# google-research/swirl-fem

Hardware: AMD Instinct MI355X
Metric: GDOF/s per CG iteration, 3D p=7 Laplacian (higher is better)
Workload: dtype f64

## Files before the change

include/sfem.h:

```cpp
#ifndef SFEM_H_
#define SFEM_H_

#include <stdint.h>

#ifdef __cplusplus
extern "C" {
#endif

#define SFEM_ABI_VERSION 10

enum { SFEM_F32 = 0, SFEM_F64 = 1 };
enum {
  SFEM_OK = 0,
  SFEM_EINVAL = -1,
  SFEM_EHIP = -2,
  SFEM_EUNSUPPORTED = -3
};
#define SFEM_SENTINEL (-1)
#define SFEM_MAX_P 16

#define SFEM_IDX_MASK 0x3FFFFFFF
#define SFEM_IDX_PAD 0x3FFFFFFF
#define SFEM_IDX_DIRICHLET 0x80000000u
#define SFEM_IDX_SHARED 0x40000000u
// ... 300 lines not shown

#define SFEM_CG_NSCALARS_NAMED 16
#define SFEM_CG_RR_SLOTS 64
#define SFEM_CG_NSCALARS (SFEM_CG_NSCALARS_NAMED + SFEM_CG_RR_SLOTS)
#define SFEM_CG_MEAN_SUMS (4 * SFEM_CG_RR_SLOTS)
#define SFEM_CG_STATUS_RUNNING 0.0
#define SFEM_CG_STATUS_CONVERGED 1.0
#define SFEM_CG_STATUS_MAXITER 2.0
#define SFEM_CG_STATUS_BAD_PAP 3.0
#define SFEM_CG_STATUS_BAD_GAMMA 4.0
int sfem_dot(const void* a, const void* b, int64_t count, double* result,
             int dtype, sfem_stream_t stream);
int sfem_dot_accumulate(const void* a, const void* b, int64_t count,
                        double* result, int dtype, sfem_stream_t stream);
int sfem_dot_indexed(const void* a, const void* b, const int64_t* idx,
                     const double* w, int64_t count, int ncomp,
                     int64_t node_stride, int64_t comp_stride, double scale,
                     double* result, int dtype, sfem_stream_t stream);
int sfem_subtract_weighted_mean(const void* w, const void* b, double total,
                                void* out, double* partials, int64_t count,
                                double* dot_result, int dtype,
                                sfem_stream_t stream);
int sfem_cg_scalars(double* scalars, int phase, double maxiter, double tol,
                    double atol, double* partials, sfem_stream_t stream);
int sfem_cg_update_xr(void* x, void* r, const void* p, const void* ap,
                      int64_t count, double* scalars, int fuse_rr, int dtype,
                      sfem_stream_t stream);
int sfem_cg_update_p(void* p, const void* z, int64_t count, double* scalars,
                     int dtype, sfem_stream_t stream);
int sfem_cg_update_r(void* r, const void* ap, int64_t count, double* scalars,
                     int fuse_rr, int dtype, sfem_stream_t stream);
int sfem_cg_update_xp(void* x, void* p, const void* z, int64_t count,
                      double* scalars, int dtype, sfem_stream_t stream);
#define SFEM_FOLD_GROUPS 256
int sfem_cg_scalars_n(double* scalars, int phase, double maxiter, double tol,
                      double atol, double* partials, int64_t num_partials,
                      sfem_stream_t stream);
int sfem_cg_update_r_layered_det(void* r, const void* ap_ext, int64_t count,
                                 const int64_t* layer_len,
                                 const int64_t* layer_off, int num_layers,
                                 const uint8_t* layer_masks,
                                 const int64_t* mask_off,
                                 double* scalars, double* rr_partials,
                                 int64_t rr_capacity, int64_t* num_rr,
                                 int dtype, sfem_stream_t stream);
#define SFEM_CG_LAZY_MAX 8
int sfem_cg_update_xp_lazy(void* x, void* pring, int64_t ring_stride,
                           const void* z, int64_t count, double* scalars,
                           double* lazy, int m, int dtype,
                           sfem_stream_t stream);
int sfem_cg_flush_x(void* x, const void* pring, int64_t ring_stride,
                    int64_t count, const double* scalars, double* lazy, int m,
                    int dtype, sfem_stream_t stream);
#define SFEM_MAX_LAYERS 15
#define SFEM_LAYER_CHUNK 512
int sfem_cg_update_r_layered(void* r, const void* ap_ext, int64_t count,
                             const int64_t* layer_len,
                             const int64_t* layer_off, int num_layers,
                             const uint8_t* layer_masks,
                             const int64_t* mask_off, double* scalars,
                             int fuse_rr, int dtype, sfem_stream_t stream);
int sfem_fold_layers(void* out_ext, int64_t count, const int64_t* layer_len,
                     const int64_t* layer_off, int num_layers, int dtype,
                     sfem_stream_t stream);
int sfem_fold_layers_at(void* out_ext, const int64_t* idx, int64_t num_idx,
                        int64_t count, const int64_t* layer_len,
                        const int64_t* layer_off, int num_layers, int dtype,
                        sfem_stream_t stream);
int sfem_cg_update_r_mean(void* r, const void* ap, const void* w,
                          int64_t count, double* scalars, double* sums,
                          int dtype, sfem_stream_t stream);
int sfem_cg_update_xp_mean(void* x, void* p, const void* r, int64_t count,
                           double* scalars, double* sums, double total,
                           int dtype, sfem_stream_t stream);
int sfem_fdm_solve(const void* r, void* z, const int64_t* pel, const void* S,
                   const int32_t* cases, const void* inv_eigenvalues,
                   int64_t num_elements, int ndim, int Pp, int dtype,
                   sfem_stream_t stream);
int sfem_fdm_solve_sums(const void* r, void* z, const int64_t* pel,
                        const void* S, const int32_t* cases,
                        const void* inv_eigenvalues, const void* weights,
                        void* elem_sum, void* weighted_sum,
                        int64_t num_elements, int ndim, int Pp, int dtype,
                        sfem_stream_t stream);
int sfem_add_element_constants(void* z, const void* yc, const void* shift,
                               int64_t num_elements, int n,
                               int64_t elems_per_member, int dtype,
                               sfem_stream_t stream);
int sfem_ell_chebyshev(const int32_t* cols, const void* vals, const void* dinv,
                       const void* b, void* x, void* work, int64_t n,
                       int width, int steps, double lmin, double lmax,
                       int dtype, sfem_stream_t stream);
#define SFEM_ENS_NSCALARS 16
#define SFEM_ENS_GROUPS 32
#define SFEM_ENS_MAX_MEMBERS 4096
int sfem_ens_dot(const void* a, const void* b, int64_t len, int members,
                 double* partials, int which, int dtype, sfem_stream_t stream);
int sfem_ens_init(double* scalars, const double* partials, int members,
                  double maxiter, double tol, double atol,
                  sfem_stream_t stream);
int sfem_ens_update_r(void* r, const void* ap, int64_t len, int members,
                      const double* scalars, const double* partials,
                      int dtype, sfem_stream_t stream);
int sfem_ens_close(double* scalars, const double* partials, int members,
                   double maxiter, sfem_stream_t stream);
int sfem_ens_update_xp(void* x, void* p, const void* z, int64_t len,
// ... 124 lines not shown
```

swirl_fem_amd/_lib.py:

```python

from __future__ import annotations

import ctypes
import os

from swirl_fem_amd import switches

_HERE = os.path.dirname(os.path.abspath(__file__))
LIB_PATH = switches.get('SFEM_LIB') or os.path.join(_HERE, 'libsfem_hip.so')
ABI_VERSION = 10

SFEM_F32, SFEM_F64 = 0, 1
SFEM_CG_NSCALARS_NAMED = 16
SFEM_CG_NSCALARS = 80
SFEM_BICGSTAB_NSCALARS = 32
BICGSTAB_STATUS = {0: 'running', 1: 'converged', 2: 'maxiter',
                   3: 'breakdown_rho', 4: 'breakdown_omega',
                   5: 'breakdown_alpha'}
CG_STATUS = {0: 'running', 1: 'converged', 2: 'maxiter', 3: 'breakdown_pAp',
             4: 'breakdown_gamma'}
SFEM_DOT_SLOTS = 1024
SFEM_CG_MEAN_SUMS = 256
SFEM_MAX_LAYERS = 15
SFEM_FOLD_GROUPS = 256
# ... 176 lines not shown
    'sfem_helmholtz_sens': [ctypes.POINTER(HelmholtzSensArgs), c_ptr],
    'sfem_facet_table_build': [c_ptr, c_ptr, c_ptr, c_ptr, c_ptr, c_i64, c_i64,
                               c_i32, c_ptr],
    'sfem_helmholtz_setup_affine': [c_ptr, c_ptr, c_i64, c_dbl, c_i32, c_ptr],
    'sfem_helmholtz_cluster_limits': [c_i32, c_i32, ctypes.POINTER(c_i32),
                                      ctypes.POINTER(c_i32)],
    'sfem_dot': [c_ptr, c_ptr, c_i64, c_ptr, c_i32, c_ptr],
    'sfem_dot_accumulate': [c_ptr, c_ptr, c_i64, c_ptr, c_i32, c_ptr],
    'sfem_dot_indexed': [c_ptr, c_ptr, c_ptr, c_ptr, c_i64, c_i32, c_i64,
                         c_i64, c_dbl, c_ptr, c_i32, c_ptr],
    'sfem_cg_scalars': [c_ptr, c_i32, c_dbl, c_dbl, c_dbl, c_ptr, c_ptr],
    'sfem_cg_update_xr': [c_ptr, c_ptr, c_ptr, c_ptr, c_i64, c_ptr, c_i32,
                          c_i32, c_ptr],
    'sfem_cg_update_p': [c_ptr, c_ptr, c_i64, c_ptr, c_i32, c_ptr],
    'sfem_cg_update_r': [c_ptr, c_ptr, c_i64, c_ptr, c_i32, c_i32, c_ptr],
    'sfem_cg_update_xp': [c_ptr, c_ptr, c_ptr, c_i64, c_ptr, c_i32, c_ptr],
    'sfem_cg_update_r_layered': [c_ptr, c_ptr, c_i64, c_ptr, c_ptr, c_i32,
                                 c_ptr, c_ptr, c_ptr, c_i32, c_i32, c_ptr],
    'sfem_kernarg_selftest': [c_ptr, c_ptr],
    'sfem_fdm_solve': [c_ptr, c_ptr, c_ptr, c_ptr, c_ptr, c_ptr, c_i64, c_i32,
                       c_i32, c_i32, c_ptr],
    'sfem_fdm_solve_sums': [c_ptr, c_ptr, c_ptr, c_ptr, c_ptr, c_ptr, c_ptr,
                            c_ptr, c_ptr, c_i64, c_i32, c_i32, c_i32, c_ptr],
    'sfem_add_element_constants': [c_ptr, c_ptr, c_ptr, c_i64, c_i32, c_i64,
                                   c_i32, c_ptr],
    'sfem_ell_chebyshev': [c_ptr, c_ptr, c_ptr, c_ptr, c_ptr, c_ptr, c_i64,
                           c_i32, c_i32, c_dbl, c_dbl, c_i32, c_ptr],
    'sfem_ens_dot': [c_ptr, c_ptr, c_i64, c_i32, c_ptr, c_i32, c_i32, c_ptr],
    'sfem_ens_init': [c_ptr, c_ptr, c_i32, c_dbl, c_dbl, c_dbl, c_ptr],
    'sfem_ens_update_r': [c_ptr, c_ptr, c_i64, c_i32, c_ptr, c_ptr, c_i32,
                          c_ptr],
    'sfem_ens_close': [c_ptr, c_ptr, c_i32, c_dbl, c_ptr],
    'sfem_ens_update_xp': [c_ptr, c_ptr, c_ptr, c_i64, c_i32, c_ptr, c_i32,
                           c_ptr],
    'sfem_ens_update_r_mean': [c_ptr, c_ptr, c_ptr, c_i64, c_i32, c_ptr, c_ptr,
                               c_ptr, c_i32, c_ptr],
    'sfem_ens_close_mean': [c_ptr, c_ptr, c_ptr, c_dbl, c_i32, c_dbl, c_ptr],
    'sfem_ens_update_xp_mean': [c_ptr, c_ptr, c_ptr, c_i64, c_i32, c_ptr,
                                c_i32, c_ptr],
    'sfem_ens_subtract_weighted_mean': [c_ptr, c_ptr, c_dbl, c_ptr, c_ptr,
                                        c_i64, c_i32, c_i32, c_ptr],
    'sfem_fold_layers': [c_ptr, c_i64, c_ptr, c_ptr, c_i32, c_i32, c_ptr],
    'sfem_fold_layers_at': [c_ptr, c_ptr, c_i64, c_i64, c_ptr, c_ptr, c_i32,
                            c_i32, c_ptr],
    'sfem_cg_scalars_n': [c_ptr, c_i32, c_dbl, c_dbl, c_dbl, c_ptr, c_i64,
                          c_ptr],
    'sfem_cg_update_r_layered_det': [c_ptr, c_ptr, c_i64, c_ptr, c_ptr, c_i32,
                                     c_ptr, c_ptr, c_ptr, c_ptr, c_i64, c_ptr,
                                     c_i32, c_ptr],
    'sfem_cg_update_xp_lazy': [c_ptr, c_ptr, c_i64, c_ptr, c_i64, c_ptr, c_ptr,
                               c_i32, c_i32, c_ptr],
    'sfem_cg_flush_x': [c_ptr, c_ptr, c_i64, c_i64, c_ptr, c_ptr, c_i32, c_i32,
                        c_ptr],
    'sfem_cg_update_r_mean': [c_ptr, c_ptr, c_ptr, c_i64, c_ptr, c_ptr, c_i32,
                              c_ptr],
    'sfem_cg_update_xp_mean': [c_ptr, c_ptr, c_ptr, c_i64, c_ptr, c_ptr, c_dbl,
                               c_i32, c_ptr],
    'sfem_axpby': [c_dbl, c_ptr, c_dbl, c_ptr, c_i64, c_i32, c_ptr],
    'sfem_helmholtz_diag': [ctypes.POINTER(DiagArgs), c_ptr],
    'sfem_cg_update_r_jacobi': [c_ptr, c_ptr, c_ptr, c_i64, c_i32, c_ptr,
                                c_ptr, c_i32, c_ptr, c_ptr, c_ptr, c_ptr,
                                c_i64, c_ptr, c_i32, c_ptr],
    'sfem_cg_update_xp_jacobi': [c_ptr, c_ptr, c_ptr, c_ptr, c_i64, c_i32,
                                 c_ptr, c_i32, c_ptr],
    'sfem_stokes_setup': [c_ptr, c_ptr, c_ptr, c_ptr, c_i64, c_i32, c_i32,
                          c_i32, c_ptr],
    'sfem_stokes_div': [c_ptr, c_ptr],
    'sfem_stokes_grad_t': [c_ptr, c_ptr],
    'sfem_stokes_e_first': [c_ptr, c_ptr],
    'sfem_stokes_e_second': [c_ptr, c_ptr],
    'sfem_stokes_convect_local': [c_ptr, c_ptr],
    'sfem_transport_rhs': [ctypes.POINTER(TransportArgs), c_ptr],
    'sfem_transport_rhs_vjp': [ctypes.POINTER(TransportVjpArgs), c_ptr],
    'sfem_point_locate': [ctypes.POINTER(PointLocateArgs), c_ptr],
    'sfem_point_eval': [ctypes.POINTER(PointArgs), c_ptr],
    'sfem_point_eval_t': [ctypes.POINTER(PointArgs), c_ptr],
    'sfem_pmg_prolong': [c_ptr, c_ptr, c_ptr, c_ptr, c_ptr, c_ptr, c_i64,
                         c_i32, c_i32, c_i32, c_i32, c_i32, c_ptr],
    'sfem_pmg_restrict': [c_ptr, c_ptr, c_ptr, c_ptr, c_ptr, c_ptr, c_i64,
                          c_i32, c_i32, c_i32, c_i32, c_ptr],
    'sfem_cheb_step': [c_ptr, c_ptr, c_ptr, c_ptr, c_ptr, c_ptr, c_dbl, c_dbl,
                       c_i64, c_i32, c_i32, c_ptr],
    'sfem_pmg_dot2': [c_ptr, c_ptr, c_ptr, c_i64, c_ptr, c_i32, c_i32, c_ptr],
    'sfem_pmg_cg_scalars': [c_ptr, c_i32, c_ptr, c_i64, c_dbl, c_dbl, c_dbl,
                            c_ptr],
    'sfem_boundary_geom': [c_ptr, c_ptr, c_i64, c_ptr, c_ptr, c_ptr, c_i32,
                           c_i32, c_i32, c_ptr, c_ptr, c_i32, c_ptr],
    'sfem_boundary_covector': [c_ptr, c_i32, c_ptr, c_i64, c_ptr, c_ptr,
                               c_i32, c_i32, c_i32, c_ptr, c_i32, c_ptr],
    'sfem_boundary_mass_apply': [c_ptr, c_ptr, c_i64, c_ptr, c_ptr, c_i32,
                                 c_i32, c_i32, c_dbl, c_ptr, c_i32, c_ptr],
    'sfem_boundary_mass_diag': [c_ptr, c_i64, c_ptr, c_ptr, c_i32, c_i32,
                                c_i32, c_dbl, c_ptr, c_i32, c_ptr],
    'sfem_boundary_add_rows': [c_ptr, c_ptr, c_ptr, c_ptr, c_i64, c_ptr, c_i32,
                               c_ptr],
    'sfem_ell_spmv': [c_ptr, c_ptr, c_ptr, c_ptr, c_i64, c_i32, c_i64, c_i64,
                      c_ptr, c_i64, c_i32, c_ptr],
    'sfem_bicgstab_scalars': [c_ptr, c_i32, c_dbl, c_dbl, c_dbl, c_ptr],
    'sfem_bicgstab_dot': [c_ptr, c_ptr, c_i64, c_ptr, c_i32, c_i32, c_i32,
                          c_ptr],
    'sfem_bicgstab_update_p': [c_ptr, c_ptr, c_ptr, c_ptr, c_ptr, c_i64, c_ptr,
                               c_i32, c_ptr],
    'sfem_bicgstab_update_s': [c_ptr, c_ptr, c_ptr, c_ptr, c_ptr, c_i64, c_ptr,
                               c_i32, c_ptr],
    'sfem_bicgstab_update_xr': [c_ptr, c_ptr, c_ptr, c_ptr, c_ptr, c_ptr,
                                c_ptr, c_i64, c_ptr, c_i32, c_ptr],
# ... 38 lines not shown
```

swirl_fem_amd/_ops.py:

```python

from __future__ import annotations

import ctypes
import os

import numpy as np
import torch

from swirl_fem_amd import switches
from swirl_fem_amd import _lib

_DT = {torch.float32: _lib.SFEM_F32, torch.float64: _lib.SFEM_F64}


def _dtype_code(t: torch.Tensor) -> int:
  try:
    return _DT[t.dtype]
  except KeyError:
    raise TypeError(f'unsupported dtype {t.dtype}; use float32 or float64')


def _dev(*tensors):
  dev = None
  for t in tensors:
# ... 499 lines not shown
    return 'sfem::helmholtz_mfma_p12_kernel<%d, %s>' % (geo_mode, b(mass))
  if part.get('cluster') is not None:
    return 'sfem::helmholtz_cluster_kernel<%s, %d, %s, %d, %s>' % (
        real, P, b(scalar), geo_mode, b(mass))
  if part.get('beta') is not None:
    return 'sfem::helmholtz_adv_kernel<%s, %d, %d, true, %d, false>' % (
        real, P, ndim, geo_mode)
  if part.get('coef_mode'):
    return ('sfem::helmholtz_kernel<%s, %d, %d, true, true, %d, false, %s, '
            '%d>' % (real, P, ndim, geo_mode, b(mass), part['coef_mode']))
  tpe = P * P if ndim == 3 else P
  can_sort = ndim == 3 and tpe <= 64
  sort = (can_sort and part.get('shared_order') is not None and
          not part.get('colored') and not (geo_mode == 3 and mass))
  b = lambda v: 'true' if v else 'false'
  return 'sfem::helmholtz_kernel<%s, %d, %d, true, %s, %d, %s, %s>' % (
      real, P, ndim, b(scalar), geo_mode, b(sort), b(mass))


def helmholtz_apply(u, out, enc, parts, host, ndim, P, lambda0, lambda1,
                    zero_range, dot_out=None, transpose=False):
  dev = _dev(enc)
  _check_vector_layout(u, out)
  host = {k: _host(v, u.dtype) for k, v in host.items()}
  if not parts and zero_range[1] > zero_range[0]:
    out[zero_range[0]:zero_range[1]].zero_()
  with torch.cuda.device(dev):
    for n, part in enumerate(parts):
      args = _helmholtz_args(u, out, part.get('enc', enc), part, host, ndim,
                             P, enc.shape[0], u.shape[0], lambda0, lambda1,
                             zero_range if n == 0 else (0, 0), dot_out,
                             transpose=transpose)
      _lib.check(_lib.load().sfem_helmholtz_apply(ctypes.byref(args),
                                                  _stream(dev)),
                 'sfem_helmholtz_apply')
  return out


def layered_dot_waves(parts, P, num_elements):
  waves = (P * P + 63) // 64
  out = []
  for part in parts:
    if part.get('layered_chains'):
      groups = part['chains'][0].numel() - 1
    elif 'elem_list' in part:
      groups = part['elem_list'].numel()
    else:
      groups = num_elements
    out.append(groups * waves)
  return out


def helmholtz_apply_layered(u, ext, enc, parts, host, ndim, P, lambda0,
                            lambda1, dot_out=None, per_wave=False):
  dev = _dev(enc)
  if u.dim() != 1 or not u.is_contiguous() or not ext.is_contiguous():
    raise ValueError('layered assembly takes contiguous scalar fields')
  if ext.dtype != u.dtype:
    raise ValueError('u and the extended output differ in dtype')
  host = {k: _host(v, u.dtype) for k, v in host.items()}
  waves = (layered_dot_waves(parts, P, enc.shape[0])
           if per_wave and dot_out is not None else None)
  if waves is not None and sum(waves) > dot_out.numel():
    raise ValueError(f'{sum(waves)} waves but {dot_out.numel()} dot slots')
  at = 0
  with torch.cuda.device(dev):
    for n, part in enumerate(parts):
      dots = dot_out if waves is None else dot_out[at:at + waves[n]]
      args = _helmholtz_args(u, ext, enc, part, host, ndim, P, enc.shape[0],
                             u.shape[0], lambda0, lambda1, (0, 0), dots,
                             layered_extent=ext.numel(),
                             dot_slots=0 if waves is None else waves[n])
      if waves is not None:
        at += waves[n]
      _lib.check(_lib.load().sfem_helmholtz_apply(ctypes.byref(args),
                                                  _stream(dev)),
                 'sfem_helmholtz_apply')
  return ext


def _layer_arrays(layers):
  n = len(layers)
  arr = ctypes.c_int64 * max(n, 1)
  return (arr(*[int(l[0]) for l in layers]) if n else arr(0),
          arr(*[int(l[1]) for l in layers]) if n else arr(0), n)


def _mask_args(masks, n):
  if masks is None:
    return None, None
  data, offs = masks
  arr = ctypes.c_int64 * max(n, 1)
  return _ptr(data), arr(*[int(o) for o in offs])


def cg_update_r_layered(r, ap_ext, layers, scalars, fuse_rr, masks=None):
  dev = _dev(r, ap_ext, scalars)
  ln, off, n = _layer_arrays(layers)
  mptr, moff = _mask_args(masks, n)
  with torch.cuda.device(dev):
    _lib.check(_lib.load().sfem_cg_update_r_layered(
        _ptr(r), _ptr(ap_ext), r.numel(), ln, off, n, mptr, moff,
        _ptr(scalars), int(fuse_rr), _dtype_code(r), _stream(dev)),
        'sfem_cg_update_r_layered')


def cg_update_r_layered_det(r, ap_ext, layers, scalars, rr_partials,
                            masks=None):
  dev = _dev(r, ap_ext, scalars, rr_partials)
  ln, off, n = _layer_arrays(layers)
  mptr, moff = _mask_args(masks, n)
  count = ctypes.c_int64(0)
  with torch.cuda.device(dev):
    _lib.check(_lib.load().sfem_cg_update_r_layered_det(
        _ptr(r), _ptr(ap_ext), r.numel(), ln, off, n, mptr, moff,
        _ptr(scalars),
        _ptr(rr_partials), rr_partials.numel(), ctypes.byref(count),
        _dtype_code(r), _stream(dev)), 'sfem_cg_update_r_layered_det')
  return count.value


def cg_scalars_n(scalars, phase, maxiter, tol, atol, partials, num_partials):
  dev = _dev(scalars, partials)
  with torch.cuda.device(dev):
    _lib.check(_lib.load().sfem_cg_scalars_n(
        _ptr(scalars), phase, float(maxiter), float(tol), float(atol),
        _ptr(partials), int(num_partials), _stream(dev)), 'sfem_cg_scalars_n')
# ... 688 lines not shown
  fn = (_lib.load().sfem_dot_accumulate if accumulate
        else _lib.load().sfem_dot)
  with torch.cuda.device(dev):
    _lib.check(fn(_ptr(a), _ptr(b), a.numel(),
                  ctypes.c_void_p(result.data_ptr() + 8 * slot),
                  _dtype_code(a), _stream(dev)), 'sfem_dot')


def dot_indexed(a, b, idx, w, result, slot, scale):
  ncomp, ns, cs = _node_view(a)
  if _node_view(b) != (ncomp, ns, cs) or a.dtype != b.dtype:
    raise ValueError('dot_indexed: operands must share layout and dtype')
  flat = lambda t: t.movedim(-1, 0) if is_component_major(t) else t
  dev = _dev(flat(a), flat(b), idx, w, result)
  with torch.cuda.device(dev):
    _lib.check(_lib.load().sfem_dot_indexed(
        _ptr(a), _ptr(b), _ptr(idx), _ptr(w), idx.numel(), ncomp, ns, cs,
        float(scale), result.data_ptr() + 8 * slot, _dtype_code(a),
        _stream(dev)), 'sfem_dot_indexed')


def cg_scalars(scalars, phase, maxiter, tol, atol, partials=None):
  dev = _dev(scalars, partials)
  with torch.cuda.device(dev):
    _lib.check(_lib.load().sfem_cg_scalars(
        _ptr(scalars), phase, float(maxiter), float(tol), float(atol),
        _ptr(partials), _stream(dev)), 'sfem_cg_scalars')


def cg_update_xr(x, r, p, ap, scalars, fuse_rr):
  dev = _dev(x, r, p, ap, scalars)
  with torch.cuda.device(dev):
    _lib.check(_lib.load().sfem_cg_update_xr(
        _ptr(x), _ptr(r), _ptr(p), _ptr(ap), x.numel(), _ptr(scalars),
        int(fuse_rr), _dtype_code(x), _stream(dev)), 'sfem_cg_update_xr')


def cg_update_p(p, z, scalars):
  dev = _dev(p, z, scalars)
  with torch.cuda.device(dev):
    _lib.check(_lib.load().sfem_cg_update_p(
        _ptr(p), _ptr(z), p.numel(), _ptr(scalars), _dtype_code(p),
        _stream(dev)), 'sfem_cg_update_p')


def cg_update_r(r, ap, scalars, fuse_rr):
  dev = _dev(r, ap, scalars)
  with torch.cuda.device(dev):
    _lib.check(_lib.load().sfem_cg_update_r(
        _ptr(r), _ptr(ap), r.numel(), _ptr(scalars), int(fuse_rr),
        _dtype_code(r), _stream(dev)), 'sfem_cg_update_r')


def cg_update_xp_lazy(x, pring, z, scalars, lazy):
  dev = _dev(x, pring, z, scalars, lazy)
  with torch.cuda.device(dev):
    _lib.check(_lib.load().sfem_cg_update_xp_lazy(
        _ptr(x), _ptr(pring), pring.stride(0), _ptr(z), x.numel(),
        _ptr(scalars), _ptr(lazy), pring.shape[0], _dtype_code(x),
        _stream(dev)), 'sfem_cg_update_xp_lazy')


def cg_flush_x(x, pring, scalars, lazy):
  dev = _dev(x, pring, scalars, lazy)
  with torch.cuda.device(dev):
    _lib.check(_lib.load().sfem_cg_flush_x(
        _ptr(x), _ptr(pring), pring.stride(0), x.numel(), _ptr(scalars),
        _ptr(lazy), pring.shape[0], _dtype_code(x), _stream(dev)),
        'sfem_cg_flush_x')


def cg_update_xp(x, p, z, scalars):
  dev = _dev(x, p, z, scalars)
  with torch.cuda.device(dev):
    _lib.check(_lib.load().sfem_cg_update_xp(
        _ptr(x), _ptr(p), _ptr(z), x.numel(), _ptr(scalars), _dtype_code(x),
        _stream(dev)), 'sfem_cg_update_xp')


def cg_update_r_mean(r, ap, w, scalars, sums):
  dev = _dev(r, ap, w, scalars, sums)
  with torch.cuda.device(dev):
    _lib.check(_lib.load().sfem_cg_update_r_mean(
        _ptr(r), _ptr(ap), _ptr(w), r.numel(), _ptr(scalars), _ptr(sums),
        _dtype_code(r), _stream(dev)), 'sfem_cg_update_r_mean')


def cg_update_xp_mean(x, p, r, scalars, sums, total):
  dev = _dev(x, p, r, scalars, sums)
  with torch.cuda.device(dev):
    _lib.check(_lib.load().sfem_cg_update_xp_mean(
        _ptr(x), _ptr(p), _ptr(r), x.numel(), _ptr(scalars), _ptr(sums),
        float(total), _dtype_code(x), _stream(dev)), 'sfem_cg_update_xp_mean')


def axpby(a, x, b, y):
  dev = _dev(x, y)
  with torch.cuda.device(dev):
    _lib.check(_lib.load().sfem_axpby(
        float(a), _ptr(x), float(b), _ptr(y), x.numel(), _dtype_code(x),
        _stream(dev)), 'sfem_axpby')
  return y


def bicgstab_scalars(scalars, phase, maxiter, tol, atol):
  dev = _dev(scalars)
  with torch.cuda.device(dev):
    _lib.check(_lib.load().sfem_bicgstab_scalars(
        _ptr(scalars), int(phase), float(maxiter), float(tol), float(atol),
        _stream(dev)), 'sfem_bicgstab_scalars')


def bicgstab_dot(a, b, scalars, slot, two=False):
# ... 257 lines not shown
```

swirl_fem_amd/core/operators.py:

```python

from __future__ import annotations

import dataclasses
import os

import numpy as np
import torch

from swirl_fem_amd import switches
from swirl_fem_amd import _ops
from swirl_fem_amd.core import autodiff

MAX_FUSED_P = 12


def supports_fused(fespace) -> str | None:
  P = fespace.mesh.gridpoints_1d.num_points
  if not fespace.is_collocated:
    return 'quadrature points differ from the nodes'
  if fespace.mesh.ndim not in (2, 3):
    return f'ndim={fespace.mesh.ndim}'
  if not 2 <= P <= MAX_FUSED_P:
    return f'P={P} outside 2..{MAX_FUSED_P}'
  d = fespace.interpolator._differentiation_matrix_1d()
# ... 161 lines not shown
    return None
  every = torch.arange(E, device=ok.device)
  cst = None
  out = []
  P = mesh.gridpoints_1d.num_points
  seg_len = chain_segment_length(E)

  def add(part, ids, mode, facet):
    if ids.numel() == 0:
      return
    new = {k: v for k, v in part.items() if k != 'elem_list'}
    new['geo_mode'] = mode
    if ids.numel() < E:
      new['elem_list'] = ids.to(torch.int32).contiguous()
    if facet:
      new.pop('shared_order', None)
      new['facet_table'] = tab
      new['geo_const'] = cst
      if seg_len > 1 and (P <= 8 or (
          switches.get('SFEM_CHAIN_HI') == '1' and
          mode in (_GEO_BOX, _GEO_AFFINE))):
        new['chains'] = facet_chains(mesh.elements, ids, P, seg_len)
        new['chain_len'] = seg_len
    out.append(new)

  use_box = switches.get('SFEM_BOX') != '0'
  for part in parts:
    ids = every if 'elem_list' not in part else part['elem_list'].long()
    good = ok[ids]
    mode = part['geo_mode']
    if mode == _GEO_MULTILINEAR and P >= 9:
      good = torch.zeros_like(good)
    if mode == _GEO_AFFINE:
      if cst is None:
        cst = _ops.helmholtz_setup_affine(coef, BOX_TOL[fespace.dtype])
      box = (cst[ids, 7] != 0) & good if use_box else torch.zeros_like(good)
      add(part, ids[box], _GEO_BOX, True)
      add(part, ids[good & ~box], _GEO_AFFINE, True)
    else:
      add(part, ids[good], mode, True)
    add(part, ids[~good], mode, False)
  return out


@dataclasses.dataclass(eq=False)
class LayerPlan:
  layers: list
  extent: int
  parts: list
  written: int
  num_nodes: int
  masks: tuple | None = None
  read: int = 0


def build_layer_plan(facet_parts, num_elements, num_nodes, P):
  from swirl_fem_amd import _lib
  if not facet_parts or any('facet_table' not in q for q in facet_parts):
    return None
  tab = facet_parts[0]['facet_table']
  dev = tab.device
  E, N = num_elements, num_nodes
  use_chains = switches.get('SFEM_CHAIN') != '0'
  has_succ = torch.zeros(E, dtype=torch.bool, device=dev)
  covered = torch.zeros(E, dtype=torch.int32, device=dev)
  for q in facet_parts:
    if q['facet_table'] is not tab:
      return None
    if 'elem_list' in q:
      covered[q['elem_list'].long()] += 1
    else:
      covered += 1
    if 'chains' in q and use_chains:
      off, elems = q['chains']
      succ = torch.ones(elems.numel(), dtype=torch.bool, device=dev)
      succ[off[1:].long() - 1] = False
      has_succ[elems.long()] = succ
  if not bool((covered == 1).all()):
    return None
  t = tab.to(torch.int64)
  code = t[..., 0] & 0xFFFFFFFF
  id0, dflag = code & 0x3FFFFFFF, code & 0x80000000
  strides = t[..., 1:]
  if int(strides[..., 1:].abs().max()) >= 32768:
    return None
  f = torch.arange(27, device=dev)
  inner = torch.stack([f // 9 == 1, (f // 3) % 3 == 1, f % 3 == 1], dim=1)
  span = strides * (P - 3) * inner[None].to(torch.int64)
  lo = id0 + span.clamp(max=0).sum(-1)
  hi = id0 + span.clamp(min=0).sum(-1) + 1
  count = torch.where(inner, P - 2, 1).prod(dim=1)
  writer = torch.ones((E, 27), dtype=torch.bool, device=dev)
  writer[:, 18:] &= ~has_succ[:, None]
  idx = torch.nonzero(writer.reshape(-1)).reshape(-1)
  key, perm = torch.sort(lo.reshape(-1)[idx], stable=True)
  first = torch.ones_like(key, dtype=torch.bool)
  first[1:] = key[1:] != key[:-1]
  pos = torch.arange(key.numel(), device=dev)
  start = torch.cummax(torch.where(first, pos, torch.zeros_like(pos)), 0).values
  layer = torch.zeros(E * 27, dtype=torch.int64, device=dev)
  layer[idx[perm]] = pos - start
  nl = int(layer.max())
  if nl > _lib.SFEM_MAX_LAYERS:
    return None
  hi_w = torch.where(writer, hi, torch.zeros_like(hi)).reshape(-1)
  lens = [int(hi_w[layer == k].max()) for k in range(1, nl + 1)]
  for k in range(nl - 2, -1, -1):
    lens[k] = max(lens[k], lens[k + 1])
  pad = lambda v: (v + 3) // 4 * 4
  lens = [pad(v) for v in lens]
  offs, at = [], pad(N)
  for v in lens:
    offs.append(at)
    at += v
  extent = at
  if extent > 0x3FFFFFFF:
    return None
  base = torch.tensor([0] + offs, dtype=torch.int64, device=dev)
  pos_out = (base[layer].reshape(E, 27) + id0) | dflag
  packed = (strides[..., 1] & 0xFFFF) | ((strides[..., 2] & 0xFFFF) << 16)
  wrap = lambda v: ((v + (1 << 31)) % (1 << 32) - (1 << 31)).to(torch.int32)
  tab2 = torch.stack([t[..., 0].to(torch.int32), wrap(pos_out),
                      strides[..., 0].to(torch.int32), wrap(packed)],
                     dim=-1).contiguous()
  written = int((writer.to(torch.int64) * count[None]).sum())
  parts = [dict(q, layered_table=tab2, layered_chains=use_chains and
                'chains' in q) for q in facet_parts]
  chunk = _lib.SFEM_LAYER_CHUNK
  flat_layer, flat_w = layer, writer.reshape(-1)
  lo_f, hi_f = lo.reshape(-1), hi.reshape(-1)
  bytes_, moffs, read = [], [], 0
  for k, ln in enumerate(lens, start=1):
    nc = (ln + chunk - 1) // chunk
    sel = flat_w & (flat_layer == k)
    first, last = lo_f[sel] // chunk, (hi_f[sel] - 1) // chunk
    d = torch.zeros(nc + 1, dtype=torch.int64, device=dev)
    d.index_add_(0, first, torch.ones_like(first))
    d.index_add_(0, last + 1, -torch.ones_like(last))
    m = (torch.cumsum(d, 0)[:nc] > 0).to(torch.uint8)
    moffs.append(sum(b.numel() for b in bytes_))
    bytes_.append(m)
    read += min(int(m.sum()) * chunk, ln)
  masks = (torch.cat(bytes_), moffs) if bytes_ else None
  return LayerPlan(layers=list(zip(lens, offs)), extent=extent, parts=parts,
                   written=written, num_nodes=N, masks=masks, read=read)


def _cluster_limits(fespace):
  mesh = fespace.mesh
  if mesh.ndim != 3:
    return None
  return _ops.helmholtz_cluster_limits(mesh.gridpoints_1d.num_points,
                                       fespace.dtype)


def _attach_clusters(fespace, enc, multiplicity, parts):
  from swirl_fem_amd.core import clusters
  size, kmax = _cluster_limits(fespace)
  ids = [None if 'elem_list' not in p else p['elem_list'].to(torch.int64)
         for p in parts]
  plans = clusters.build_cluster_plan(fespace.mesh, enc, multiplicity, ids,
                                      size, kmax)
  out = []
  for part, plan in zip(parts, plans):
    if plan is not None:
      out.append(dict({k: v for k, v in part.items() if k != 'shared_order'},
                      cluster=plan))
  return out


def colored_launch_order(colors, num_colors, group, num_groups):
  colors = colors.to(torch.int64)
  group = group.to(torch.int64)
  out = []
  for c in range(num_colors):
    for g in range(num_groups):
      lst = torch.nonzero((colors == c) & (group == g)).reshape(-1)
      if lst.numel():
        out.append((g, lst))
  return out


def first_toucher_violations(elements, first, launches):
  el = elements.to(torch.int64)
  E = el.shape[0]
  launch = torch.full((E,), -1, dtype=torch.int64, device=el.device)
  for i, (_, lst) in enumerate(launches):
    launch[lst.to(device=el.device, dtype=torch.int64)] = i
  ok = el >= 0
  if not bool(ok.any()):
    return 0
  if bool((launch[ok.any(dim=1)] < 0).any()):
    raise RuntimeError('coloured assembly: an element is in no launch')
  slot_launch = launch[:, None].expand_as(el)
  num_nodes = int(el[ok].max()) + 1
  first_launch = torch.full((num_nodes,), -1, dtype=torch.int64,
                            device=el.device)
  first_launch.scatter_reduce_(0, el[first & ok], slot_launch[first & ok],
# ... 489 lines not shown
                                        _diag=None, _diag_adv=None,
                                        _geo_parts=geo))
    return tuple(halves)

  def apply(self, u, lambda0=0.0, lambda1=1.0, out=None, *, zero=True,
            dot_out=None, _transpose=False):
    mesh = self.fespace.mesh
    if u.shape[0] != mesh.num_nodes:
      raise ValueError(f'expected {mesh.num_nodes} nodal values, got '
                       f'{tuple(u.shape)}')
    if self.coefs is not None:
      _check_scalar_field(u)
      lambda0, lambda1 = _scaled(self.coefs, lambda0, lambda1)
    if self.beta is not None:
      _check_scalar_field(u, 'a velocity takes')
      if dot_out is not None:
        raise NotImplementedError('dot_out of an operator with a velocity')
    u = u.to(self.fespace.dtype)
    if not (u.is_contiguous() or _ops.is_component_major(u)):
      u = u.contiguous()
    if out is None:
      out = torch.empty_like(u)
    return _ops.helmholtz_apply(
        u, out, self.enc, self._parts_for(u), self.host, mesh.ndim,
        mesh.gridpoints_1d.num_points, lambda0, lambda1,
        self.zero_range if zero else (0, 0), dot_out, transpose=_transpose)

  def apply_transpose(self, u, lambda0=0.0, lambda1=1.0, out=None):
    if self.beta is None:
      return self.apply(u, lambda0, lambda1, out)
    return self.apply(u, lambda0, lambda1, out, _transpose=True)

  def sensitivity(self, u, lam, lambda0=0.0, lambda1=1.0,
                  want=(True, True, True)):
    return _sensitivity(self, u, lam, lambda0, lambda1, want)

  def layer_plan(self):
    if self._layer_plan is None:
      plan = None
      if (self.facet_parts is not None and
          switches.get('SFEM_LAYERED') != '0'):
        mesh = self.fespace.mesh
        plan = build_layer_plan(self.facet_parts, mesh.num_elements,
                                mesh.num_nodes, mesh.gridpoints_1d.num_points)
      self._layer_plan = plan if plan is not None else False
    return self._layer_plan or None

  def new_extended(self):
    plan = self.layer_plan()
    return torch.zeros(plan.extent, dtype=self.fespace.dtype,
                       device=self.enc.device)

  def apply_layered(self, u, ext, lambda0=0.0, lambda1=1.0, *, dot_out=None,
                    per_wave=False):
    plan = self.layer_plan()
    if plan is None:
      raise NotImplementedError('this operator has no layer plan')
    mesh = self.fespace.mesh
    if tuple(u.shape) != (mesh.num_nodes,):
      raise ValueError(f'expected ({mesh.num_nodes},) nodal values, got '
                       f'{tuple(u.shape)}')
    if tuple(ext.shape) != (plan.extent,):
      raise ValueError(f'expected an extended output of {plan.extent} values')
    return _ops.helmholtz_apply_layered(
        u.to(self.fespace.dtype).contiguous(), ext, self.enc, plan.parts,
        self.host, mesh.ndim, mesh.gridpoints_1d.num_points, lambda0, lambda1,
        dot_out, per_wave)

  def layered_dot_slots(self):
    mesh = self.fespace.mesh
    return sum(_ops.layered_dot_waves(self.layer_plan().parts,
                                      mesh.gridpoints_1d.num_points,
                                      mesh.num_elements))

  def _parts_for(self, u):
    if self.facet_parts is None or not (
        u.dim() == 1 or u.shape[-1] == 1 or _ops.is_component_major(u)):
      return self.parts
    if u.dim() == 1 or u.shape[-1] == 1:
      return self.facet_parts
    if self._vector_parts is None:
      if not any(q['geo_mode'] == _GEO_POINT and 'facet_table' in q
                 for q in self.facet_parts):
        self._vector_parts = self.facet_parts
      elif self.fespace.dtype == torch.float64:
        self._vector_parts = (
            [q for q in self.facet_parts if q['geo_mode'] != _GEO_POINT] +
            [q for q in self.parts if q['geo_mode'] == _GEO_POINT])
      else:
        self._vector_parts = [
            {k: v for k, v in q.items() if k != 'chains'}
            if q['geo_mode'] == _GEO_POINT else q for q in self.facet_parts]
    return self._vector_parts

  def diagonal(self, lambda0=0.0, lambda1=1.0, assembled=True):
    return _diagonal(self, self.keep, None, lambda0, lambda1, assembled)

  def point_weights(self):
    return _point_weights(self)

  def apply_local(self, u_local, lambda0=0.0, lambda1=1.0, *,
                  transpose=False):
    mesh = self.fespace.mesh
    if self.coefs is not None:
      if u_local.dim() == 3 and u_local.shape[-1] != 1:
        raise NotImplementedError('coefficients take scalar fields')
      lambda0, lambda1 = _scaled(self.coefs, lambda0, lambda1)
    if self.beta is not None and u_local.dim() == 3 and u_local.shape[-1] != 1:
      raise NotImplementedError('a velocity takes scalar fields')
    return _ops.helmholtz_local(
        u_local.to(self.fespace.dtype), self.parts, self.host, mesh.ndim,
        mesh.gridpoints_1d.num_points, lambda0, lambda1,
        transpose=transpose and self.beta is not None)

  def linear_operator(self, lambda0=0.0, lambda1=1.0, transpose=False):
    if self.beta is not None:
      return _PlainLinearOperator(self, lambda0, lambda1, transpose)
    return FusedLinearOperator(self, lambda0, lambda1)

  def bytes_per_apply(self, lambda0=0.0, ncomp=1, layered=False):
    mesh = self.fespace.mesh
    E, n = mesh.elements.shape
    s = 8 if self.fespace.dtype == torch.float64 else 4
    total = 2 * s * mesh.num_nodes * ncomp
    parts = self.facet_parts if self.facet_parts is not None else self.parts
    if layered:
      plan = self.layer_plan()
      total = s * (mesh.num_nodes + plan.written)
      parts = plan.parts
    for part in parts:
      count = part['elem_list'].numel() if 'elem_list' in part else E
      mode = part['geo_mode']
      if 'facet_table' in part:
        conn = 27 * 16 + (4 if 'chains' in part and ncomp == 1 else 0)
      else:
        conn = 4 * n + (4 if 'elem_list' in part else 0)
        if part.get('shared_order') is not None:
          conn += 2 * part['shared_order'].shape[1]
      if mode == _GEO_POINT:
        geo = (7 if lambda0 else 6) * s * n
      elif 'facet_table' in part and mode in (_GEO_AFFINE, _GEO_BOX):
        geo = 8 * s
      else:
        geo = 24 * s
      geo += _coefficient_bytes(part, s, n, lambda0)
      if part.get('beta') is not None:
        geo += s * n * mesh.ndim
      total += count * (conn + geo)
    return total

  def kernel_name(self, lambda0=0.0, lambda1=1.0, ncomp=1, layered=False):
    mesh = self.fespace.mesh
    real = 'double' if self.fespace.dtype == torch.float64 else 'float'
    P = mesh.gridpoints_1d.num_points
    names = []
    parts = (self.layer_plan().parts if layered else
             self.parts if self.facet_parts is None else self.facet_parts)
    for part in parts:
      gm = part['geo_mode']
      names.append(_ops.helmholtz_kernel_name(
          real, P, mesh.ndim, ncomp == 1, gm, part,
          _scaled(self.coefs, lambda0, lambda1)[0] != 0, layered))
    return ' + '.join(sorted(set(names)))


class FusedLinearOperator:

  def __init__(self, op, lambda0, lambda1):
    self.op, self.lambda0, self.lambda1 = op, lambda0, lambda1
    self._ext = None

  def __call__(self, u):
    return self.op.apply(u, self.lambda0, self.lambda1)

  def apply_with_dot(self, u, partials):
    return self.op.apply(u, self.lambda0, self.lambda1, dot_out=partials)

  def layer_plan(self):
    plan = self.op.layer_plan()
    if plan is not None and switches.get('SFEM_LAYERED') != 'force' and any(
        q['geo_mode'] == _GEO_POINT for q in plan.parts):
      return None
    return plan

  def apply_layered_with_dot(self, u, partials, per_wave=False):
    if self._ext is None:
      self._ext = self.op.new_extended()
    return self.op.apply_layered(u, self._ext, self.lambda0, self.lambda1,
                                 dot_out=partials, per_wave=per_wave)

  def layered_dot_slots(self):
    return self.op.layered_dot_slots()


def supports_fused_stokes(vspace, pspace) -> str | None:
  why = supports_fused(vspace)
  if why is not None:
    return why
  P = vspace.mesh.gridpoints_1d.num_points
  if P < 4:
    return f'P={P} < 4'
  if pspace.mesh.gridpoints_1d.num_points != P - 2:
    return 'pressure space is not P - 2 points per direction'
  if pspace.interpolator.evalpoints_1d != vspace.mesh.gridpoints_1d:
    return 'pressure quadrature differs from the velocity nodes'
  if pspace.mesh.num_elements != vspace.mesh.num_elements:
    return 'velocity and pressure meshes have different elements'
  E = vspace.mesh.num_elements
  sample = torch.unique(torch.linspace(
      0, max(E - 1, 0), steps=min(E, 512), device=vspace.device).round().long())
  jv, jp = _sample_jacdets(vspace, sample), _sample_jacdets(pspace, sample)
  ndim = vspace.mesh.ndim
  if jv.numel():
    h = 2.0 * float(jv.abs().amax()) ** (1.0 / ndim)
    xmax = float(vspace.mesh.node_coords.abs().amax())
    P = vspace.mesh.gridpoints_1d.num_points
    rounding = 32 * torch.finfo(jv.dtype).eps * P * P * max(xmax / h, 1.0)
  else:
    rounding = 0.0
  tight = 1e-10 if jv.dtype == torch.float64 else 1e-4
  kind = _cached_geometry_kind(vspace)[sample]
  tol = torch.where(kind != _GEO_POINT, max(tight, rounding),
                    max(tight, rounding / 4)).to(jv.dtype)
  if jv.shape != jp.shape or not bool(
      ((jv - jp).abs() <= tol[:, None] * jv.abs().amax()).all()):
    return 'velocity and pressure spaces carry different geometry'
  return None


def _cached_geometry_kind(fespace):
  cache = fespace._cache
  if 'geometry_kind' not in cache:
    cache['geometry_kind'] = classify_geometry(fespace)[0]
  return cache['geometry_kind']


def _sample_jacdets(space, elements):
  mesh = space.mesh
  i1, g1 = space._matrices()
  xe = _ops.gather_rows(mesh.node_coords,
                        mesh.elements[elements].contiguous())
  _, jacdets, _ = _ops.geom_factors(
# ... 629 lines not shown
```

swirl_fem_amd/csrc/sfem_common.h:

```cpp
#pragma once
#include <hip/hip_runtime.h>
#include <stdint.h>
#include <stdio.h>

#include "sfem.h"

namespace sfem {

void set_error(const char* fmt, ...);

inline hipStream_t as_stream(sfem_stream_t s) {
  return reinterpret_cast<hipStream_t>(s);
}

#define SFEM_REQUIRE(cond, ...)          \
  do {                                   \
    if (!(cond)) {                       \
      ::sfem::set_error(__VA_ARGS__);    \
      return SFEM_EINVAL;                \
    }                                    \
  } while (0)

#define SFEM_HIP(call)                                                   \
  do {                                                                   \
    hipError_t err__ = (call);                                           \
    if (err__ != hipSuccess) {                                           \
      ::sfem::set_error("%s failed: %s", #call, hipGetErrorString(err__)); \
      return SFEM_EHIP;                                                  \
    }                                                                    \
  } while (0)

#define SFEM_LAUNCH_CHECK()                                              \
  do {                                                                   \
    hipError_t err__ = hipGetLastError();                                \
    if (err__ != hipSuccess) {                                           \
      ::sfem::set_error("kernel launch failed: %s",                      \
                        hipGetErrorString(err__));                       \
      return SFEM_EHIP;                                                  \
    }                                                                    \
  } while (0)

inline unsigned stream_grid(int64_t work_items, int block) {
  int64_t blocks = (work_items + block - 1) / block;
  const int64_t cap = 256 * 128;
  if (blocks > cap) blocks = cap;
  if (blocks < 1) blocks = 1;
  return static_cast<unsigned>(blocks);
}

inline bool streams_past_caches(int64_t count, size_t elem_size) {
  return (size_t)count * elem_size >= ((size_t)256 << 20);
}

inline unsigned reduce_grid(int64_t work_items, int block) {
  int64_t blocks = (work_items + block - 1) / block;
  const int64_t cap = 256 * 16;
  if (blocks > cap) blocks = cap;
  if (blocks < 1) blocks = 1;
  return static_cast<unsigned>(blocks);
}

}
```

swirl_fem_amd/csrc/sfem_core.hip:

```cpp
#include <stdarg.h>
#include <string.h>

#include "sfem_common.h"

namespace sfem {

static thread_local char g_error[512] = "";

void set_error(const char* fmt, ...) {
  va_list ap;
  va_start(ap, fmt);
  vsnprintf(g_error, sizeof(g_error), fmt, ap);
  va_end(ap);
}

template <typename T>
__global__ void __launch_bounds__(256)
gather_kernel(const T* __restrict__ u, const int32_t* __restrict__ idx,
              T* __restrict__ out, int64_t count, T fill) {
  const int64_t stride = (int64_t)gridDim.x * blockDim.x;
  for (int64_t i = (int64_t)blockIdx.x * blockDim.x + threadIdx.x; i < count;
       i += stride) {
    const int32_t k = idx[i];
    out[i] = k < 0 ? fill : u[k];
// ... 312 lines not shown
    acc += (double)a[i] * (double)b[i];
  const double total = block_sum(acc);
  if (threadIdx.x == 0) partials[blockIdx.x] = total;
}

template <typename T>
__global__ void __launch_bounds__(512)
subtract_mean_kernel(const T* __restrict__ w, const double* __restrict__ partials,
                     int num_partials, double inv_total, T* __restrict__ out,
                     int64_t count, double* __restrict__ dot_result) {
  __shared__ double mean;
  double acc = 0.0;
  for (int i = threadIdx.x; i < num_partials; i += blockDim.x)
    acc += partials[i];
  const double total = block_sum(acc);
  if (threadIdx.x == 0) mean = total * inv_total;
  __syncthreads();
  const T m = (T)mean;
  const int64_t stride = (int64_t)gridDim.x * blockDim.x;
  double wz = 0.0;
  for (int64_t i = (int64_t)blockIdx.x * blockDim.x + threadIdx.x; i < count;
       i += stride) {
    const T wi = w[i], zi = wi - m;
    out[i] = zi;
    wz += (double)wi * (double)zi;
  }
  if (dot_result) {
    const double tot = block_sum(wz);
    if (threadIdx.x == 0) unsafeAtomicAdd(dot_result, tot);
  }
}

template <typename T>
__global__ void __launch_bounds__(256)
dot_indexed_kernel(const T* __restrict__ a, const T* __restrict__ b,
                   const int64_t* __restrict__ idx,
                   const double* __restrict__ w, int64_t count, int ncomp,
                   int64_t node_stride, int64_t comp_stride, double scale,
                   double* __restrict__ result) {
  const int64_t stride = (int64_t)gridDim.x * blockDim.x;
  double acc = 0.0;
  for (int64_t i = (int64_t)blockIdx.x * blockDim.x + threadIdx.x; i < count;
       i += stride) {
    const int64_t k = idx[i] * node_stride;
    double s = 0.0;
    for (int c = 0; c < ncomp; ++c)
      s += (double)a[k + c * comp_stride] * (double)b[k + c * comp_stride];
    acc += w[i] * s;
  }
  const double total = block_sum(acc);
  if (threadIdx.x == 0 && total != 0.0) unsafeAtomicAdd(result, scale * total);
}

__device__ __forceinline__ double cg_gamma_new(const double* scalars) {
  double v = scalars[SFEM_CG_NSCALARS_NAMED + (threadIdx.x & 63)];
#pragma unroll
  for (int off = 32; off > 0; off >>= 1) v += __shfl_xor(v, off, 64);
  return scalars[2] + v;
}

template <typename T, bool FUSE_RR>
__global__ void __launch_bounds__(512)
cg_update_xr_kernel(T* __restrict__ x, T* __restrict__ r,
                    const T* __restrict__ p, const T* __restrict__ ap,
                    int64_t count, double* __restrict__ scalars) {
  if (scalars[7] != 0.0) return;
  using V = typename Vec16<T>::type;
  constexpr int VN = Vec16<T>::N;
  const T alpha = (T)(scalars[0] / scalars[1]);
  const int64_t nvec = count / VN;
  V* xv = reinterpret_cast<V*>(x);
  V* rv = reinterpret_cast<V*>(r);
  const V* pv = reinterpret_cast<const V*>(p);
  const V* apv = reinterpret_cast<const V*>(ap);
  const int64_t stride = (int64_t)gridDim.x * blockDim.x;
  double acc = 0.0;
  for (int64_t i = (int64_t)blockIdx.x * blockDim.x + threadIdx.x; i < nvec;
       i += stride) {
    V xx = xv[i], rr = rv[i];
    const V pp = pv[i], aa = apv[i];
#pragma unroll
    for (int c = 0; c < VN; ++c) {
      T* xe = reinterpret_cast<T*>(&xx) + c;
      T* re = reinterpret_cast<T*>(&rr) + c;
      *xe += alpha * vget<T>(pp, c);
      *re -= alpha * vget<T>(aa, c);
      if (FUSE_RR) acc += (double)*re * (double)*re;
    }
    xv[i] = xx;
    rv[i] = rr;
  }
  if (blockIdx.x == 0 && threadIdx.x < count - nvec * VN) {
    const int64_t i = nvec * VN + threadIdx.x;
    x[i] += alpha * p[i];
    const T rn = r[i] - alpha * ap[i];
    r[i] = rn;
    if (FUSE_RR) acc += (double)rn * (double)rn;
  }
  if (FUSE_RR) {
    const double total = block_sum(acc);
    if (threadIdx.x == 0) unsafeAtomicAdd(&scalars[2], total);
  }
}

template <typename T>
__global__ void __launch_bounds__(512)
cg_update_p_kernel(T* __restrict__ p, const T* __restrict__ z, int64_t count,
                   const double* __restrict__ scalars) {
  if (scalars[7] != 0.0) return;
  using V = typename Vec16<T>::type;
  constexpr int VN = Vec16<T>::N;
  const T beta = (T)(cg_gamma_new(scalars) / scalars[0]);
// ... 50 lines not shown
    if (FUSE_RR) acc += (double)rn * (double)rn;
  }
  if (FUSE_RR) {
    const double total = block_sum(acc);
    if (threadIdx.x == 0)
      unsafeAtomicAdd(STRIPED ? &scalars[SFEM_CG_NSCALARS_NAMED +
                                         (blockIdx.x & (SFEM_CG_RR_SLOTS - 1))]
                              : &scalars[2], total);
  }
}

template <typename T, bool NT>
__global__ void __launch_bounds__(512)
cg_update_xp_kernel(T* __restrict__ x, T* __restrict__ p,
                    const T* __restrict__ z, int64_t count,
                    const double* __restrict__ scalars) {
  if (scalars[7] != 0.0) return;
  using V = typename Vec16<T>::type;
  constexpr int VN = Vec16<T>::N;
  const T alpha = (T)(scalars[0] / scalars[1]);
  const T beta = (T)(cg_gamma_new(scalars) / scalars[0]);
  const int64_t nvec = count / VN;
  V* xv = reinterpret_cast<V*>(x);
  V* pv = reinterpret_cast<V*>(p);
  const V* zv = reinterpret_cast<const V*>(z);
  const int64_t stride = (int64_t)gridDim.x * blockDim.x;
  for (int64_t i = (int64_t)blockIdx.x * blockDim.x + threadIdx.x; i < nvec;
       i += stride) {
    V xx = ld16<T, NT>(&xv[i]);
    V pp = ld16<T, NT>(&pv[i]);
    const V zz = ld16<T, NT>(&zv[i]);
#pragma unroll
    for (int c = 0; c < VN; ++c) {
      T* xe = reinterpret_cast<T*>(&xx) + c;
      T* pe = reinterpret_cast<T*>(&pp) + c;
      *xe += alpha * *pe;
      *pe = vget<T>(zz, c) + beta * *pe;
    }
    st16<T, NT>(xx, &xv[i]);
    st16<T, NT>(pp, &pv[i]);
  }
  if (blockIdx.x == 0 && threadIdx.x < count - nvec * VN) {
    const int64_t i = nvec * VN + threadIdx.x;
    const T pi = p[i];
    x[i] += alpha * pi;
    p[i] = z[i] + beta * pi;
  }
}

template <typename T, bool NT>
__global__ void __launch_bounds__(512)
cg_update_xp_lazy_kernel(T* __restrict__ x, T* __restrict__ pring,
                         int64_t ring_stride, const T* __restrict__ z,
                         int64_t count, const double* __restrict__ scalars,
                         double* __restrict__ lazy, int m) {
  if (scalars[7] != 0.0) return;
  using V = typename Vec16<T>::type;
  constexpr int VN = Vec16<T>::N;
  const int64_t k = (int64_t)scalars[8];
  const int slot = (int)(k % m), next = (int)((k + 1) % m);
  const T alpha = (T)(scalars[0] / scalars[1]);
  const T beta = (T)(cg_gamma_new(scalars) / scalars[0]);
  const bool flush = next == 0;
  int64_t lo = (int64_t)lazy[0];
  if (lo < k + 1 - m) lo = k + 1 - m;
  T a_old[SFEM_CG_LAZY_MAX];
  int s_old[SFEM_CG_LAZY_MAX];
  int n_old = 0;
  if (flush) {
    for (int64_t j = lo; j < k; ++j) {
      s_old[n_old] = (int)(j % m);
      a_old[n_old++] = (T)lazy[1 + (j % m)];
    }
  }
  if (blockIdx.x == 0 && threadIdx.x == 0) lazy[1 + slot] = (double)alpha;
  const int64_t nvec = count / VN;
  V* xv = reinterpret_cast<V*>(x);
  const V* pk = reinterpret_cast<const V*>(pring + slot * ring_stride);
  V* pn = reinterpret_cast<V*>(pring + next * ring_stride);
  const V* zv = reinterpret_cast<const V*>(z);
  const int64_t stride = (int64_t)gridDim.x * blockDim.x;
  for (int64_t i = (int64_t)blockIdx.x * blockDim.x + threadIdx.x; i < nvec;
       i += stride) {
    const V pp = ld16<T, NT>(&pk[i]);
    const V zz = ld16<T, NT>(&zv[i]);
    if (flush) {
      V xx = ld16<T, NT>(&xv[i]);
      for (int q = 0; q < n_old; ++q) {
        const V po = ld16<T, NT>(
            reinterpret_cast<const V*>(pring + s_old[q] * ring_stride) + i);
#pragma unroll
        for (int c = 0; c < VN; ++c)
          reinterpret_cast<T*>(&xx)[c] += a_old[q] * vget<T>(po, c);
      }
#pragma unroll
      for (int c = 0; c < VN; ++c)
        reinterpret_cast<T*>(&xx)[c] += alpha * vget<T>(pp, c);
      st16<T, NT>(xx, &xv[i]);
    }
    V np;
#pragma unroll
    for (int c = 0; c < VN; ++c)
      reinterpret_cast<T*>(&np)[c] = vget<T>(zz, c) + beta * vget<T>(pp, c);
    st16<T, NT>(np, &pn[i]);
  }
  if (blockIdx.x == 0 && threadIdx.x < count - nvec * VN) {
    const int64_t i = nvec * VN + threadIdx.x;
    const T pi = pring[slot * ring_stride + i];
    if (flush) {
      T xx = x[i];
      for (int q = 0; q < n_old; ++q)
        xx += a_old[q] * pring[s_old[q] * ring_stride + i];
      xx += alpha * pi;
      x[i] = xx;
    }
    pring[next * ring_stride + i] = z[i] + beta * pi;
  }
}

template <typename T>
__global__ void __launch_bounds__(512)
cg_flush_x_kernel(T* __restrict__ x, const T* __restrict__ pring,
                  int64_t ring_stride, int64_t count,
                  const double* __restrict__ scalars,
                  const double* __restrict__ lazy, int m) {
  const int64_t iters = (int64_t)scalars[8];
  int64_t lo = (int64_t)lazy[0];
  if (lo < iters - iters % m) lo = iters - iters % m;
  if (lo >= iters) return;
  const int64_t stride = (int64_t)gridDim.x * blockDim.x;
  for (int64_t i = (int64_t)blockIdx.x * blockDim.x + threadIdx.x; i < count;
       i += stride) {
    T xx = x[i];
    for (int64_t j = lo; j < iters; ++j)
      xx += (T)lazy[1 + (j % m)] * pring[(j % m) * ring_stride + i];
    x[i] = xx;
  }
}

__global__ void cg_lazy_mark_kernel(const double* __restrict__ scalars,
                                    double* __restrict__ lazy) {
  if (threadIdx.x == 0 && blockIdx.x == 0) lazy[0] = scalars[8];
}

template <typename T, bool NT>
__global__ void __launch_bounds__(512)
cg_update_r_mean_kernel(T* __restrict__ r, const T* __restrict__ ap,
                        const T* __restrict__ w, int64_t count,
                        double* __restrict__ scalars,
                        double* __restrict__ sums) {
  if (scalars[7] != 0.0) return;
  using V = typename Vec16<T>::type;
  constexpr int VN = Vec16<T>::N;
  const T alpha = (T)(scalars[0] / scalars[1]);
  double* set = sums + (((int64_t)scalars[8]) & 1) * (2 * SFEM_CG_RR_SLOTS);
  const int64_t nvec = count / VN;
  V* rv = reinterpret_cast<V*>(r);
  const V* apv = reinterpret_cast<const V*>(ap);
  const V* wv = reinterpret_cast<const V*>(w);
  const int64_t stride = (int64_t)gridDim.x * blockDim.x;
  double rr_acc = 0.0, one_acc = 0.0, w_acc = 0.0;
  for (int64_t i = (int64_t)blockIdx.x * blockDim.x + threadIdx.x; i < nvec;
       i += stride) {
    V rr = ld16<T, NT>(&rv[i]);
    const V aa = ld16<T, NT>(&apv[i]);
    const V ww = ld16<T, NT>(&wv[i]);
#pragma unroll
    for (int c = 0; c < VN; ++c) {
      T* re = reinterpret_cast<T*>(&rr) + c;
      *re -= alpha * vget<T>(aa, c);
// ... 1049 lines not shown
               "sfem_cg_update_r_jacobi: %d components need a period that is "
               "a multiple of %d and no layers", ncomp, vn);
  if (num_rz) *num_rz = 0;
  if (period == 0) return SFEM_OK;
  SFEM_REQUIRE(r && ap_ext && dinv, "sfem_cg_update_r_jacobi: null pointer");
  LayerDesc ld;
  const int rc = make_layer_desc("sfem_cg_update_r_jacobi", layer_len,
                                 layer_off, num_layers, period, vn, &ld,
                                 layer_masks, mask_off);
  if (rc != SFEM_OK) return rc;
  int grid = stream_grid(period, 512 * 2);
  if (rz_partials && grid > rz_capacity) grid = (int)rz_capacity;
  if (num_rz) *num_rz = rz_partials ? grid : 0;
  DISPATCH_DTYPE(dtype, launch_update_r_jacobi<T>(
      streams_past_caches(period * ncomp, sizeof(T)), rz_partials != nullptr,
      grid, as_stream(stream), (T*)r, (const T*)ap_ext, (const T*)dinv,
      period, ncomp, ld, scalars, rz_partials));
  SFEM_LAUNCH_CHECK();
  return SFEM_OK;
}

int sfem_cg_update_xp_jacobi(void* x, void* p, const void* r,
                             const void* dinv, int64_t period, int ncomp,
                             double* scalars, int dtype,
                             sfem_stream_t stream) {
  SFEM_REQUIRE(period >= 0 && ncomp >= 1 && scalars,
               "sfem_cg_update_xp_jacobi: bad arguments");
  SFEM_REQUIRE(dtype == SFEM_F32 || dtype == SFEM_F64,
               "sfem_cg_update_xp_jacobi: unknown dtype %d", dtype);
  SFEM_REQUIRE(ncomp == 1 || period % (dtype == SFEM_F64 ? 2 : 4) == 0,
               "sfem_cg_update_xp_jacobi: %d components need a period that "
               "is a multiple of the vector width", ncomp);
  if (period == 0) return SFEM_OK;
  SFEM_REQUIRE(x && p && r && dinv, "sfem_cg_update_xp_jacobi: null pointer");
  DISPATCH_DTYPE(dtype, {
    const unsigned grid = stream_grid(period, 512 * 2);
    if (streams_past_caches(period * ncomp, sizeof(T)))
      hipLaunchKernelGGL((cg_update_xp_jacobi_kernel<T, true>), dim3(grid),
                         dim3(512), 0, as_stream(stream), (T*)x, (T*)p,
                         (const T*)r, (const T*)dinv, period, ncomp, scalars);
    else
      hipLaunchKernelGGL((cg_update_xp_jacobi_kernel<T, false>), dim3(grid),
                         dim3(512), 0, as_stream(stream), (T*)x, (T*)p,
                         (const T*)r, (const T*)dinv, period, ncomp, scalars);
  });
  SFEM_LAUNCH_CHECK();
  return SFEM_OK;
}

int sfem_cg_update_xp_lazy(void* x, void* pring, int64_t ring_stride,
                           const void* z, int64_t count, double* scalars,
                           double* lazy, int m, int dtype,
                           sfem_stream_t stream) {
  SFEM_REQUIRE(count >= 0 && scalars && lazy,
               "sfem_cg_update_xp_lazy: bad arguments");
  SFEM_REQUIRE(m >= 2 && m <= SFEM_CG_LAZY_MAX,
               "sfem_cg_update_xp_lazy: ring of %d directions (2..%d)", m,
               SFEM_CG_LAZY_MAX);
  if (count == 0) return SFEM_OK;
  SFEM_REQUIRE(x && pring && z && ring_stride >= count,
               "sfem_cg_update_xp_lazy: null pointer or ring stride < count");
  SFEM_REQUIRE(dtype == SFEM_F32 || dtype == SFEM_F64,
               "sfem_cg_update_xp_lazy: unknown dtype %d", dtype);
  SFEM_REQUIRE(ring_stride % (dtype == SFEM_F64 ? 2 : 4) == 0,
               "sfem_cg_update_xp_lazy: ring stride must keep 16-byte "
               "alignment");
  DISPATCH_DTYPE(dtype, {
    const int grid = stream_grid(count, 512 * 2);
    if (streams_past_caches(count, sizeof(T)))
      hipLaunchKernelGGL((cg_update_xp_lazy_kernel<T, true>), dim3(grid),
                         dim3(512), 0, as_stream(stream), (T*)x, (T*)pring,
                         ring_stride, (const T*)z, count, scalars, lazy, m);
    else
      hipLaunchKernelGGL((cg_update_xp_lazy_kernel<T, false>), dim3(grid),
                         dim3(512), 0, as_stream(stream), (T*)x, (T*)pring,
                         ring_stride, (const T*)z, count, scalars, lazy, m);
  });
  SFEM_LAUNCH_CHECK();
  return SFEM_OK;
}

int sfem_cg_flush_x(void* x, const void* pring, int64_t ring_stride,
                    int64_t count, const double* scalars, double* lazy, int m,
                    int dtype, sfem_stream_t stream) {
  SFEM_REQUIRE(count >= 0 && scalars && lazy && m >= 2 &&
                   m <= SFEM_CG_LAZY_MAX,
               "sfem_cg_flush_x: bad arguments");
  SFEM_REQUIRE(dtype == SFEM_F32 || dtype == SFEM_F64,
               "sfem_cg_flush_x: unknown dtype %d", dtype);
  if (count > 0) {
    SFEM_REQUIRE(x && pring && ring_stride >= count,
                 "sfem_cg_flush_x: null pointer or ring stride < count");
    DISPATCH_DTYPE(dtype, {
      hipLaunchKernelGGL((cg_flush_x_kernel<T>),
                         dim3(stream_grid(count, 512)), dim3(512), 0,
                         as_stream(stream), (T*)x, (const T*)pring,
                         ring_stride, count, scalars, lazy, m);
    });
  }
  hipLaunchKernelGGL(cg_lazy_mark_kernel, dim3(1), dim3(1), 0,
                     as_stream(stream), scalars, lazy);
  SFEM_LAUNCH_CHECK();
  return SFEM_OK;
}

int sfem_cg_update_r_mean(void* r, const void* ap, const void* w,
                          int64_t count, double* scalars, double* sums,
                          int dtype, sfem_stream_t stream) {
  SFEM_REQUIRE(count >= 0 && scalars && sums,
               "sfem_cg_update_r_mean: bad arguments");
  if (count == 0) return SFEM_OK;
  SFEM_REQUIRE(r && ap && w, "sfem_cg_update_r_mean: null pointer");
  DISPATCH_DTYPE(dtype, {
    const int grid = stream_grid(count, 512 * 2);
    if (streams_past_caches(count, sizeof(T)))
      hipLaunchKernelGGL((cg_update_r_mean_kernel<T, true>), dim3(grid),
                         dim3(512), 0, as_stream(stream), (T*)r, (const T*)ap,
                         (const T*)w, count, scalars, sums);
    else
      hipLaunchKernelGGL((cg_update_r_mean_kernel<T, false>), dim3(grid),
                         dim3(512), 0, as_stream(stream), (T*)r, (const T*)ap,
                         (const T*)w, count, scalars, sums);
  });
  SFEM_LAUNCH_CHECK();
  return SFEM_OK;
}

int sfem_cg_update_xp_mean(void* x, void* p, const void* r, int64_t count,
                           double* scalars, double* sums, double total,
// ... 68 lines not shown
```

swirl_fem_amd/csrc/sfem_helmholtz.hip:

```cpp
#include <stdlib.h>

#include "sfem_helmholtz_cluster.h"
#include "sfem_helmholtz_mfma.h"
#include "sfem_helmholtz_facet.h"
#include "sfem_helmholtz_adv.h"
#include "sfem_helmholtz_sens.h"

namespace sfem {

template <typename T>
__global__ void __launch_bounds__(256)
helmholtz_setup_kernel(const T* __restrict__ invjac,
                       const T* __restrict__ jacdet,
                       const T* __restrict__ weights, T* __restrict__ geo,
                       int64_t num_elements, int d, int Q) {
  const int ng = d * (d + 1) / 2;
  const int64_t total = num_elements * Q;
  const int64_t stride = (int64_t)gridDim.x * blockDim.x;
  for (int64_t t = (int64_t)blockIdx.x * blockDim.x + threadIdx.x; t < total;
       t += stride) {
    const int64_t e = t / Q;
    const int q = (int)(t - e * Q);
    const T* ij = invjac + t * d * d;
    const T wd = weights[q] * jacdet[t];
// ... 159 lines not shown
  }
  __syncthreads();
  for (int s = lane; s < n; s += 64) {
    const int a = s / (P * P), i = (s / P) % P, j = s % P;
    const int f = cls(a) * 9 + cls(i) * 3 + cls(j);
    const uint32_t code = (uint32_t)ent[f][0];
    const int32_t pred = (int32_t)(code & SFEM_IDX_MASK) + ent[f][1] * (a - 1) +
                         ent[f][2] * (i - 1) + ent[f][3] * (j - 1);
    const int32_t id = ids[s];
    bool good = id == pred && id >= 0 && id < num_nodes;
    if (good) {
      const bool dir = dirichlet && dirichlet[id];
      const bool sh = multiplicity[id] > 1;
      good = dir == ((code & SFEM_IDX_DIRICHLET) != 0) &&
             sh == ((code & SFEM_IDX_SHARED) != 0);
    }
    if (!good) atomicOr(&bad, 1);
  }
  __syncthreads();
  if (lane < 27) {
    int32_t* dst = tab + e * FACET_ROW + lane * 4;
    for (int q = 0; q < 4; ++q) dst[q] = ent[lane][q];
  }
  if (lane == 0) ok[e] = bad ? 0 : 1;
}

struct HelmholtzCall {
  const void* u; void* out; const int32_t* enc; const void* geo;
  const void* geo_elem; const int32_t* geo_index; const int32_t* elem_list;
  const void* dmat; const void* weights; const void* nodes;
  int64_t num_elements; int ndim, P, ncomp, geo_mode; double l0, l1; bool gs;
  double* dot_out;
  int colored;
  int64_t node_stride, comp_stride;
  const uint16_t* shared_order = nullptr;
  int shared_stride = 0;
  const int32_t* cluster_elems = nullptr;
  const int32_t* cluster_offsets = nullptr;
  const uint32_t* cluster_nodes = nullptr;
  int64_t num_clusters = 0;
  const int32_t* facet_table = nullptr;
  const void* geo_const = nullptr;
  int64_t num_nodes = 0;
  const int32_t* chain_offsets = nullptr;
  const int32_t* chain_elems = nullptr;
  int64_t num_chains = 0;
  int64_t layered_extent = 0;
  int64_t dot_slots = 0;
  const void* kappa = nullptr;
  const void* sigma = nullptr;
  int coef_mode = 0;
  const void* beta = nullptr;
  int adv_transpose = 0;
};

template <typename T>
static int run_helmholtz(const HelmholtzCall& c, hipStream_t stream) {
  HelmholtzParams<T> prm{};
  prm.u = (const T*)c.u; prm.out = (T*)c.out; prm.enc = c.enc;
  prm.geo = (const T*)c.geo; prm.geo_elem = (const T*)c.geo_elem;
  prm.geo_index = c.geo_index; prm.geo_mode = c.geo_mode;
  prm.dmat_host = (const T*)c.dmat; prm.weights_host = (const T*)c.weights;
  prm.nodes_host = (const T*)c.nodes; prm.num_elements = c.num_elements;
  prm.elem_list = c.elem_list; prm.ncomp = c.ncomp;
  prm.node_stride = c.node_stride > 0 ? c.node_stride : c.ncomp;
  prm.comp_stride = c.node_stride > 0 ? c.comp_stride : 1;
  prm.comp = 0; prm.lambda0 = (T)c.l0; prm.lambda1 = (T)c.l1;
  prm.dot_out = c.dot_out;
  prm.colored = c.colored;
  prm.shared_order = c.shared_order;
  prm.shared_stride = c.shared_stride;
  if (c.beta) {
    HelmholtzAdvParams<T> ap{};
    static_cast<HelmholtzParams<T>&>(ap) = prm;
    ap.dot_out = nullptr;
    ap.shared_order = nullptr;
    ap.kappa = (const T*)c.kappa;
    ap.sigma = (const T*)c.sigma;
    ap.beta = (const T*)c.beta;
    const bool tr = c.adv_transpose != 0;
    return with_dim(c.ndim, [&](auto d) {
      return dispatch_helmholtz_adv<T, decltype(d)::value>(ap, c.P, c.gs, tr,
                                                           stream);
    });
  }
  if (c.coef_mode != COEF_NONE) {
    HelmholtzCoefParams<T> cp{};
    static_cast<HelmholtzParams<T>&>(cp) = prm;
    cp.kappa = (const T*)c.kappa;
    cp.sigma = (const T*)c.sigma;
    cp.coef_mode = c.coef_mode;
    return with_dim(c.ndim, [&](auto d) {
      return dispatch_helmholtz_coef<T, decltype(d)::value>(cp, c.P, c.gs,
                                                            stream);
    });
  }
  if (c.cluster_elems) {
    ClusterParams<T> cl{c.cluster_elems, c.cluster_offsets, c.cluster_nodes,
                        c.num_clusters};
    return dispatch_helmholtz_cluster<T>(prm, cl, c.P, stream);
  }
  if (c.facet_table) {
    FacetParams<T> fp{};
    fp.u = prm.u; fp.out = prm.out; fp.tab = c.facet_table;
    fp.geo_const = (const T*)c.geo_const; fp.geo_elem = prm.geo_elem;
    fp.geo = prm.geo; fp.geo_index = prm.geo_index;
    fp.elem_list = prm.elem_list; fp.comp_stride = prm.comp_stride;
    fp.ncomp = prm.ncomp; fp.lambda0 = prm.lambda0; fp.lambda1 = prm.lambda1;
    fp.dot_out = prm.dot_out;
    fp.chain_off = c.chain_offsets;
    fp.chain_elems = c.chain_elems;
    fp.layered = c.layered_extent > 0;
    fp.dot_slots = c.dot_slots;
    if (fp.layered)
      return dispatch_helmholtz_facet<T>(
          fp, c.P, c.geo_mode,
          c.chain_offsets ? c.num_chains : c.num_elements, c.layered_extent,
          prm.dmat_host, prm.weights_host, prm.nodes_host, stream);
    if (c.chain_offsets && c.ncomp > 1) {
      for (int k = 0; k < c.ncomp; ++k) {
        FacetParams<T> fk = fp;
        fk.u = prm.u + (int64_t)k * prm.comp_stride;
        fk.out = prm.out + (int64_t)k * prm.comp_stride;
        fk.ncomp = 1;
        const int rc = dispatch_helmholtz_facet<T>(
            fk, c.P, c.geo_mode, c.num_chains, c.num_nodes, prm.dmat_host,
            prm.weights_host, prm.nodes_host, stream);
        if (rc != SFEM_OK) return rc;
      }
      return SFEM_OK;
    }
    return dispatch_helmholtz_facet<T>(fp, c.P, c.geo_mode,
                                       c.chain_offsets ? c.num_chains
                                                       : c.num_elements,
                                       c.num_nodes, prm.dmat_host,
                                       prm.weights_host, prm.nodes_host,
                                       stream);
  }
  if constexpr (sizeof(T) == 4) {
    const char* v = getenv("SFEM_MFMA");
    const bool mfma_on = v && v[0] == '1';
    if (mfma_on && helmholtz_mfma_applies(prm, c.P, c.ndim, c.gs))
      return launch_helmholtz_mfma_p12(prm, stream);
  }
  if (c.ndim == 3) return dispatch_helmholtz<T, 3>(prm, c.P, c.gs, stream);
  if (c.ndim == 2) return dispatch_helmholtz<T, 2>(prm, c.P, c.gs, stream);
  set_error("helmholtz: ndim=%d (fused kernel supports 2 and 3)", c.ndim);
  return SFEM_EUNSUPPORTED;
}

static int check_coefficients(const char* who, const sfem_helmholtz_args* a) {
  if (a->coef_mode == SFEM_COEF_NONE) return SFEM_OK;
  SFEM_REQUIRE(a->coef_mode == SFEM_COEF_ELEM || a->coef_mode == SFEM_COEF_POINT,
               "%s: unknown coef_mode %d", who, a->coef_mode);
  SFEM_REQUIRE(a->kappa || a->sigma,
               "%s: coef_mode %d needs kappa or sigma", who, a->coef_mode);
  SFEM_REQUIRE(a->ncomp == 1, "%s: coefficients take scalar fields", who);
  SFEM_REQUIRE(a->ndim == 2 || a->ndim == 3, "%s: coefficients need ndim 2 or 3",
               who);
  SFEM_REQUIRE(a->geo_mode == SFEM_GEO_AFFINE ||
                   a->geo_mode == SFEM_GEO_MULTILINEAR,
               "%s: coefficients need affine or multilinear elements (fold "
               "them into the stored factors of curved ones)", who);
  SFEM_REQUIRE(!a->cluster_elems && !a->facet_table && !a->shared_order &&
                   !a->layered_extent,
               "%s: coefficients run on index rows (no cluster, facet, "
// ... 43 lines not shown
  hipLaunchKernelGGL((kernarg_probe_kernel<PRM, MAT>), dim3(1), dim3(64), 0,
                     st, prm, mat, bad);
}

}

using namespace sfem;

extern "C" {

int sfem_helmholtz_setup(const void* invjac, const void* jacdet,
                         const void* weights_nd, void* geo,
                         int64_t num_elements, int ndim, int Q, int dtype,
                         sfem_stream_t stream) {
  SFEM_REQUIRE(num_elements >= 0 && ndim >= 1 && ndim <= 3 && Q >= 1,
               "sfem_helmholtz_setup: bad sizes");
  if (num_elements == 0) return SFEM_OK;
  SFEM_REQUIRE(invjac && jacdet && weights_nd && geo,
               "sfem_helmholtz_setup: null pointer");
  const unsigned grid = stream_grid(num_elements * Q, 256);
  if (dtype == SFEM_F64)
    hipLaunchKernelGGL(helmholtz_setup_kernel<double>, dim3(grid), dim3(256), 0,
                       as_stream(stream), (const double*)invjac,
                       (const double*)jacdet, (const double*)weights_nd,
                       (double*)geo, num_elements, ndim, Q);
  else if (dtype == SFEM_F32)
    hipLaunchKernelGGL(helmholtz_setup_kernel<float>, dim3(grid), dim3(256), 0,
                       as_stream(stream), (const float*)invjac,
                       (const float*)jacdet, (const float*)weights_nd,
                       (float*)geo, num_elements, ndim, Q);
  else {
    set_error("sfem_helmholtz_setup: unknown dtype %d", dtype);
    return SFEM_EINVAL;
  }
  SFEM_LAUNCH_CHECK();
  return SFEM_OK;
}

int sfem_encode_elements(const int32_t* elements, const uint8_t* dirichlet,
                         const int32_t* multiplicity,
                         const uint8_t* slot_shared, int32_t* enc,
                         int64_t count, sfem_stream_t stream) {
  SFEM_REQUIRE(count >= 0, "sfem_encode_elements: negative count");
  if (count == 0) return SFEM_OK;
  SFEM_REQUIRE(elements && (multiplicity || slot_shared) && enc,
               "sfem_encode_elements: null pointer");
  hipLaunchKernelGGL(encode_kernel, dim3(stream_grid(count, 256)), dim3(256), 0,
                     as_stream(stream), elements, dirichlet, multiplicity,
                     slot_shared, enc, count);
  SFEM_LAUNCH_CHECK();
  return SFEM_OK;
}

int sfem_helmholtz_apply(const sfem_helmholtz_args* a, sfem_stream_t stream) {
  SFEM_REQUIRE(a, "sfem_helmholtz_apply: null args");
  SFEM_REQUIRE(a->num_elements >= 0 && a->num_nodes >= 0 && a->ncomp >= 1 &&
                   a->ncomp <= 8,
               "sfem_helmholtz_apply: bad sizes");
  SFEM_REQUIRE(a->dtype == SFEM_F32 || a->dtype == SFEM_F64,
               "sfem_helmholtz_apply: unknown dtype %d", a->dtype);
  SFEM_REQUIRE(a->num_nodes <= SFEM_IDX_MASK,
               "sfem_helmholtz_apply: more than 2^30-1 nodes per device");
  SFEM_REQUIRE(0 <= a->zero_begin && a->zero_begin <= a->zero_end &&
                   a->zero_end <= a->num_nodes,
               "sfem_helmholtz_apply: bad zero range");
  if (a->num_nodes == 0) return SFEM_OK;
  SFEM_REQUIRE(a->out, "sfem_helmholtz_apply: null out");
  const size_t esz = a->dtype == SFEM_F64 ? 8 : 4;
  if (a->zero_end > a->zero_begin) {
    int rc0;
    if (a->node_stride > 0 && a->node_stride != a->ncomp) {
      SFEM_REQUIRE(a->node_stride == 1,
                   "sfem_helmholtz_apply: unsupported vector layout");
      rc0 = sfem_zero_strips((char*)a->out + (size_t)a->zero_begin * esz,
                             a->zero_end - a->zero_begin, a->comp_stride,
                             a->ncomp, a->dtype, stream);
    } else {
      rc0 = sfem_zero_strips(
          (char*)a->out + (size_t)a->zero_begin * a->ncomp * esz,
          (a->zero_end - a->zero_begin) * a->ncomp, 0, 1, a->dtype, stream);
    }
    if (rc0) return rc0;
  }
  if (a->num_elements == 0) return SFEM_OK;
  SFEM_REQUIRE(a->u && (a->enc || a->facet_table) && a->dmat,
               "sfem_helmholtz_apply: null pointer");
  SFEM_REQUIRE(a->geo_mode != SFEM_GEO_BOX || a->facet_table,
               "sfem_helmholtz_apply: SFEM_GEO_BOX needs a facet table");
  int rc = check_geometry("sfem_helmholtz_apply", a->geo_mode, a->geo, "geo",
                          a->geo_elem, a->weights, a->nodes);
  if (rc) return rc;
  rc = check_advection("sfem_helmholtz_apply", a);
  if (rc) return rc;
  rc = check_coefficients("sfem_helmholtz_apply", a);
  if (rc) return rc;
  int64_t work;
  rc = check_elem_list("sfem_helmholtz_apply", a->elem_list, a->num_listed,
                       a->num_elements, &work);
  if (rc) return rc;
  if (work == 0) return SFEM_OK;
  HelmholtzCall c{a->u, a->out, a->enc, a->geo, a->geo_elem, a->geo_index,
                  a->elem_list, a->dmat, a->weights, a->nodes, work, a->ndim,
                  a->P, a->ncomp, a->geo_mode, a->lambda0, a->lambda1, true,
                  a->dot_out, a->colored, a->node_stride, a->comp_stride,
                  a->shared_order, a->shared_stride};
  c.kappa = a->kappa;
  c.sigma = a->sigma;
// ... 9 lines not shown
    SFEM_REQUIRE(a->cluster_offsets && a->cluster_nodes && a->num_clusters > 0,
                 "sfem_helmholtz_apply: incomplete cluster description");
    SFEM_REQUIRE(!a->colored && !a->shared_order,
                 "sfem_helmholtz_apply: clusters exclude colored / "
                 "shared_order");
    c.cluster_elems = a->cluster_elems;
    c.cluster_offsets = a->cluster_offsets;
    c.cluster_nodes = a->cluster_nodes;
    c.num_clusters = a->num_clusters;
  }
  if (a->facet_table) {
    SFEM_REQUIRE(a->ndim == 3 && facet_supported_p(a->P),
                 "sfem_helmholtz_apply: facet tables are 3D, P = 6..12");
    SFEM_REQUIRE(!a->colored && !a->cluster_elems,
                 "sfem_helmholtz_apply: facet tables exclude colored / "
                 "cluster assembly");
    SFEM_REQUIRE(a->ncomp == 1 || a->node_stride == 1,
                 "sfem_helmholtz_apply: facet tables need node_stride = 1");
    SFEM_REQUIRE(a->geo_const || (a->geo_mode != SFEM_GEO_AFFINE &&
                                  a->geo_mode != SFEM_GEO_BOX),
                 "sfem_helmholtz_apply: affine / box facet applies need "
                 "geo_const");
    c.facet_table = a->facet_table;
    c.geo_const = a->geo_const;
    c.num_nodes = a->num_nodes;
    if (a->layered_extent) {
      SFEM_REQUIRE(a->layered_extent >= a->num_nodes &&
                       a->layered_extent <= SFEM_IDX_MASK,
                   "sfem_helmholtz_apply: layered_extent must cover the "
                   "nodal values and stay below 2^30");
      SFEM_REQUIRE(a->ncomp == 1 && a->zero_end == a->zero_begin,
                   "sfem_helmholtz_apply: layered assembly takes scalar "
                   "fields and clears nothing");
      c.layered_extent = a->layered_extent;
      SFEM_REQUIRE(a->dot_slots >= 0, "sfem_helmholtz_apply: negative dot_slots");
      c.dot_slots = a->dot_slots;
    } else {
      SFEM_REQUIRE(a->dot_slots == 0,
                   "sfem_helmholtz_apply: dot_slots goes with layered "
                   "assembly");
    }
    if (a->chain_offsets) {
      SFEM_REQUIRE(a->chain_elems && a->num_chains > 0 &&
                       (a->ncomp == 1 || a->node_stride == 1),
                   "sfem_helmholtz_apply: chains need chain_elems, "
                   "num_chains > 0 and a scalar or component-major field");
      c.chain_offsets = a->chain_offsets;
      c.chain_elems = a->chain_elems;
      c.num_chains = a->num_chains;
    }
  }
  SFEM_REQUIRE(!a->layered_extent || a->facet_table,
               "sfem_helmholtz_apply: layered assembly needs a facet table");
  return with_real(a->dtype, [&](auto zero) {
    return run_helmholtz<decltype(zero)>(c, as_stream(stream));
  });
}

int sfem_kernarg_selftest(int32_t* bad, sfem_stream_t stream) {
  SFEM_REQUIRE(bad, "sfem_kernarg_selftest: null pointer");
  hipStream_t st = as_stream(stream);
  launch_kernarg_probe<FacetParams<double>, SMat<double, 8>>(bad, st);
  launch_kernarg_probe<FacetParams<double>, DMat<double, 8>>(bad, st);
  launch_kernarg_probe<FacetParams<float>, DMat<float, 12>>(bad, st);
  launch_kernarg_probe<FacetParams<float>, SMat<float, 12>>(bad, st);
  SFEM_LAUNCH_CHECK();
  return SFEM_OK;
}

int sfem_facet_table_build(const int32_t* elements, const uint8_t* dirichlet,
                           const int32_t* multiplicity, int32_t* table,
                           uint8_t* ok, int64_t num_elements,
                           int64_t num_nodes, int P, sfem_stream_t stream) {
  SFEM_REQUIRE(num_elements >= 0 && num_nodes >= 0 && P >= 2 && P <= 12,
               "sfem_facet_table_build: bad sizes");
  if (num_elements == 0) return SFEM_OK;
  SFEM_REQUIRE(elements && multiplicity && table && ok,
               "sfem_facet_table_build: null pointer");
  SFEM_REQUIRE(num_elements <= 0x7fffffff,
               "sfem_facet_table_build: too many elements");
  hipLaunchKernelGGL(facet_table_kernel, dim3((unsigned)num_elements), dim3(64),
                     0, as_stream(stream), elements, dirichlet, multiplicity,
                     table, ok, num_elements, num_nodes, P);
  SFEM_LAUNCH_CHECK();
  return SFEM_OK;
}

int sfem_helmholtz_setup_affine(const void* geo_elem, void* geo_const,
                                int64_t num_elements, double box_tol,
                                int dtype, sfem_stream_t stream) {
  SFEM_REQUIRE(num_elements >= 0, "sfem_helmholtz_setup_affine: bad sizes");
  if (num_elements == 0) return SFEM_OK;
  SFEM_REQUIRE(geo_elem && geo_const,
               "sfem_helmholtz_setup_affine: null pointer");
  const unsigned grid = (unsigned)((num_elements + 255) / 256);
  if (dtype == SFEM_F64)
    hipLaunchKernelGGL(helmholtz_setup_affine_kernel<double>, dim3(grid),
                       dim3(256), 0, as_stream(stream),
                       (const double*)geo_elem, (double*)geo_const,
                       num_elements, box_tol);
  else if (dtype == SFEM_F32)
    hipLaunchKernelGGL(helmholtz_setup_affine_kernel<float>, dim3(grid),
                       dim3(256), 0, as_stream(stream), (const float*)geo_elem,
                       (float*)geo_const, num_elements, (float)box_tol);
  else {
    set_error("sfem_helmholtz_setup_affine: unknown dtype %d", dtype);
    return SFEM_EINVAL;
  }
  SFEM_LAUNCH_CHECK();
// ... 131 lines not shown
```

swirl_fem_amd/csrc/sfem_helmholtz_facet.h:

```cpp
#pragma once
#include <stdlib.h>

#include "sfem_helmholtz.h"

namespace sfem {

constexpr int FACET_ROW = 27 * 4;

template <typename T>
struct FacetParams {
  const T* u;
  T* out;
  const int32_t* tab;
  const T* geo_const;
  const T* geo_elem;
  const T* geo;
  const int32_t* geo_index;
  const int32_t* elem_list;
  const int32_t* chain_off;
  const int32_t* chain_elems;
  int64_t comp_stride;
  int ncomp;
  T lambda0, lambda1;
  double* dot_out;
  int layered;
  int64_t dot_slots;
};

constexpr uint32_t FACET_SKIP = 0x40000000u;

template <int P>
struct FacetLayout {
  static constexpr int B = P >= 9 ? (P | 1) : P;
  static constexpr int A = P == 8 ? 67 : (P == 7 ? 52 : P * B);
  static constexpr bool SWAP = P == 8;
  static constexpr int WORDS = (P - 1) * (A + B + 1) + 1;
  static constexpr int COPY = (WORDS + 3) & ~3;
  static constexpr int TPE = P * P;
  static constexpr int WAVES = (TPE + 63) / 64;
  static constexpr int BLOCK = 64 * WAVES;
  __host__ __device__ static constexpr int word(int x, int y, int z) {
    return A * x + B * y + z;
  }
};

template <int P>
__device__ __forceinline__ void facet_sync() {
  if (FacetLayout<P>::WAVES == 1) wave_sync();
  else lds_barrier();
}

template <int P>
struct FacetSlots {
  uint16_t s[FacetLayout<P>::BLOCK][6];
};

template <int P>
constexpr FacetSlots<P> make_facet_slots() {
  using L = FacetLayout<P>;
  FacetSlots<P> t{};
  for (int l = 0; l < L::BLOCK; ++l)
    for (int q = 0; q < 6; ++q) t.s[l][q] = 0xFFFF;
  constexpr int M = P - 2, NF = M * M;
  static_assert(NF + 2 * M + 8 <= L::TPE, "rounds must fit the element's lanes");
  int edges[12][3] = {};
  int ne = 0;
  for (int d = 2; d >= 0; --d)
    for (int pp = 0; pp < 2; ++pp)
      for (int r = 0; r < 2; ++r) {
        int c[3] = {0, 0, 0};
        c[d] = -1;
        c[(d + 1) % 3] = pp ? P - 1 : 0;
        c[(d + 2) % 3] = r ? P - 1 : 0;
        for (int k = 0; k < 3; ++k) edges[ne][k] = c[k];
        ++ne;
      }
  for (int q = 0; q < 6; ++q) {
    const int d = q / 2, fixed = (q & 1) ? P - 1 : 0;
    for (int l = 0; l < NF; ++l) {
      const int x = l / M + 1, y = l % M + 1;
      int c[3] = {0, 0, 0};
      c[d] = fixed;
      c[(d + 1) % 3] = d == 1 ? y : x;
      c[(d + 2) % 3] = d == 1 ? x : y;
      t.s[l][q] = (uint16_t)L::word(c[0], c[1], c[2]);
    }
    for (int h = 0; h < 2; ++h)
      for (int z = 0; z < M; ++z) {
        int c[3] = {0, 0, 0};
        for (int k = 0; k < 3; ++k)
          c[k] = edges[2 * q + h][k] < 0 ? z + 1 : edges[2 * q + h][k];
        t.s[NF + h * M + z][q] = (uint16_t)L::word(c[0], c[1], c[2]);
      }
  }
  for (int v = 0; v < 8; ++v)
    t.s[NF + 2 * M + v][0] = (uint16_t)L::word(
        (v & 4) ? P - 1 : 0, (v & 2) ? P - 1 : 0, (v & 1) ? P - 1 : 0);
// ... 169 lines not shown
  }
}

template <typename T, int P, bool OFF32>
__device__ __forceinline__ void facet_scatter_tail(
    const FacetLane<P>& fl, const uint16_t (&slots)[6], const T (&acc)[P],
    T* og, T* vals, uint32_t* codes, uint32_t own_w, bool lane_ok) {
  using L = FacetLayout<P>;
#pragma unroll
  for (int c = 0; c < 3; ++c) {
    if (lane_ok && !(fl.t[c] & SFEM_IDX_SHARED)) {
#pragma unroll
      for (int a = 0; a < P; ++a)
        if (FacetLane<P>::cls(a) == c) {
          *facet_node<T, OFF32>(og, fl.code(a)) = acc[a];
        }
    }
  }
  if (lane_ok) {
#pragma unroll
    for (int a = 0; a < P; ++a) {
      vals[own_w + a * L::A] = acc[a];
      codes[own_w + a * L::A] = fl.code(a);
    }
  }
  facet_sync<P>();
#pragma unroll
  for (int q = 0; q < 6; ++q) {
    const uint32_t w = slots[q];
    if (w != 0xFFFFu) {
      const uint32_t code = codes[w];
      if ((code & ~(uint32_t)SFEM_IDX_MASK) == SFEM_IDX_SHARED) {
        unsafeAtomicAdd(facet_node<T, OFF32>(og, code), vals[w]);
      }
    }
  }
}

template <typename T, int P, bool OFF32>
__device__ __forceinline__ void facet_store_layered(
    const FacetLane<P, true>& fl, const T (&acc)[P], T* og, bool lane_ok) {
#pragma unroll
  for (int c = 0; c < 3; ++c) {
    if (lane_ok && !(fl.to[c] & FACET_SKIP)) {
#pragma unroll
      for (int a = 0; a < P; ++a)
        if (FacetLane<P, true>::cls(a) == c)
          *facet_node<T, OFF32>(og, fl.ocode(a)) = acc[a];
    }
  }
}

template <typename T, int P, bool OFF32>
__device__ __forceinline__ void facet_store_layered_slots(
    const FacetLane<P, true>& fl, const uint16_t (&slots)[6], const T (&acc)[P],
    T* og, T* vals, uint32_t* codes, uint32_t own_w, bool lane_ok,
    bool inner_lane) {
  using L = FacetLayout<P>;
  if (lane_ok && inner_lane) {
#pragma unroll
    for (int a = 1; a < P - 1; ++a)
      *facet_node<T, OFF32>(og, fl.ocode(a)) = acc[a];
  }
  if (lane_ok) {
#pragma unroll
    for (int a = 0; a < P; ++a) {
      vals[own_w + a * L::A] = acc[a];
      codes[own_w + a * L::A] = fl.ocode(a);
    }
  }
  facet_sync<P>();
#pragma unroll
  for (int q = 0; q < 6; ++q) {
    const uint32_t w = slots[q];
    if (w != 0xFFFFu) {
      const uint32_t code = codes[w];
      if (!(code & FACET_SKIP)) *facet_node<T, OFF32>(og, code) = vals[w];
    }
  }
}

template <typename PRM, typename MAT>
struct FacetKernarg {
  static constexpr size_t MAT_OFF =
      (sizeof(PRM) + alignof(MAT) - 1) / alignof(MAT) * alignof(MAT);
};

__device__ __forceinline__ const char* kernarg_bytes() {
#if defined(__HIP_DEVICE_COMPILE__)
  return (const char*)(const __attribute__((address_space(4))) char*)
      __builtin_amdgcn_kernarg_segment_ptr();
#else
  return nullptr;
#endif
}

#ifndef SFEM_FACET_AFFINE_MINW
#define SFEM_FACET_AFFINE_MINW 5
#endif
#ifndef SFEM_FACET_BOX_MINW
#define SFEM_FACET_BOX_MINW 5
#endif
#ifndef SFEM_FACET_BOX_MINW_HI
#define SFEM_FACET_BOX_MINW_HI 3
#endif
#ifndef SFEM_FACET_CHAIN_MINW_HI
#define SFEM_FACET_CHAIN_MINW_HI 2
#endif
#ifndef SFEM_FACET_CHAIN_MINW_GEN
#define SFEM_FACET_CHAIN_MINW_GEN 3
#endif
#ifndef SFEM_FACET_CHAIN_MINW_BOX
#define SFEM_FACET_CHAIN_MINW_BOX 4
#endif
#ifndef SFEM_FACET_CHAIN_MINW_AFFINE
#define SFEM_FACET_CHAIN_MINW_AFFINE 4
#endif

template <typename T, int P, typename M>
__device__ __forceinline__ T sym_w(const M& m, int a) {
  return m.w[a < P - 1 - a ? a : P - 1 - a];
}

template <typename T, int P, bool TRANS, typename PRM>
__device__ __forceinline__ void facet_line(const DMat<T, P>& dm,
                                           const T (&x)[P], T (&y)[P]) {
  if constexpr (P >= 9 && sizeof(T) == 4) {
    using KA = FacetKernarg<PRM, DMat<T, P>>;
    line_apply_mem<T, P, TRANS>(
        (const SFEM_CONSTANT_AS DMat<T, P>*)((const SFEM_CONSTANT_AS char*)
                                                 __builtin_amdgcn_kernarg_segment_ptr() +
                                             KA::MAT_OFF),
// ... 8 lines not shown
                                               const T (&x)[P], T (&y)[P]) {
  if constexpr (P >= 9 && sizeof(T) == 4) {
    using KA = FacetKernarg<PRM, SMat<T, P>>;
    sym_line_apply_mem<T, P>(
        (const SFEM_CONSTANT_AS SMat<T, P>*)((const SFEM_CONSTANT_AS char*)
                                                 __builtin_amdgcn_kernarg_segment_ptr() +
                                             KA::MAT_OFF),
        x, y);
  } else {
    sym_line_apply<T, P>(sm, x, y);
  }
}

template <int P>
struct FacetWave {
  using L = FacetLayout<P>;
  static constexpr int TPE = P * P;
  int lane, i, j;
  bool ok;
  uint32_t own_w, mid_w, last_w;
  template <typename T, typename M>
  __device__ __forceinline__ T wij(const M* kmat) const {
    return kmat->w[i] * kmat->w[j];
  }
  __device__ __forceinline__ void init() {
    lane = threadIdx.x;
    ok = TPE == L::BLOCK || lane < TPE;
    const int t = ok ? lane : 0;
    i = t / P;
    j = t - i * P;
    own_w = L::B * i + j;
    mid_w = L::SWAP ? L::A * j + i : L::A * i + j;
    last_w = L::SWAP ? L::A * j + L::B * i : L::A * i + L::B * j;
  }
};

template <typename T, int P, int GM, bool MASS>
struct FacetElem {
  using L = FacetLayout<P>;
  using Mat = DMat<T, P>;
  static constexpr int LDS_WORDS = 2 * L::COPY;
  static constexpr int MINW =
      P >= 9 ? 2 : (GM == GEO_AFFINE ? SFEM_FACET_AFFINE_MINW : 4);
  static constexpr int CHAIN_MINW =
      P >= 9 ? 2 : (GM == GEO_AFFINE ? SFEM_FACET_CHAIN_MINW_AFFINE
                                    : SFEM_FACET_CHAIN_MINW_GEN);
  static constexpr bool CHAINS = GM == GEO_AFFINE || P <= 8;
  static constexpr bool LAYERED_SLOTS = P <= 8 && GM != GEO_MULTILINEAR;
  struct Raw { T c[GM == GEO_AFFINE ? 7 : 1]; int64_t e; };
  T cst[GM == GEO_AFFINE ? 6 : 1];
  T lw, Wm0;
  ElemGeom<T, P, 3, (GM == GEO_AFFINE ? GEO_POINT : GM)> geom;

  static __device__ __forceinline__ void fetch(Raw& raw,
                                               const FacetParams<T>& prm,
                                               int64_t e) {
    raw.e = e;
    if constexpr (GM == GEO_AFFINE) {
      const T* g = prm.geo_const + e * 8;
#pragma unroll
      for (int q = 0; q < 7; ++q) raw.c[q] = g[q];
    }
  }
  __device__ __forceinline__ void finish(const Raw& raw,
                                         const FacetParams<T>& prm,
                                         const Mat& dm, const Mat* kdm,
                                         const FacetWave<P>& w, T wij) {
    lw = T(0);
    Wm0 = T(0);
    if constexpr (GM == GEO_AFFINE) {
#pragma unroll
      for (int q = 0; q < 6; ++q) cst[q] = raw.c[q];
      lw = prm.lambda1 * wij;
      if (MASS) Wm0 = prm.lambda0 * raw.c[6] * wij;
    } else {
      HelmholtzParams<T> hp{};
      hp.geo = prm.geo;
      hp.geo_elem = prm.geo_elem;
      hp.geo_index = prm.geo_index;
      geom.template init<true>(hp, dm, raw.e, true, w.i, w.j,
                               w.ok ? w.lane : 0, kdm);
    }
  }

  __device__ __forceinline__ void apply(const FacetParams<T>& prm,
                                        const Mat& dm, const FacetWave<P>& w,
                                        T* lds, const T (&ua)[P],
                                        T (&acc)[P]) const {
    T* s0 = lds;
    T* s1 = lds + L::COPY;
    const bool lane_ok = w.ok;
    const uint32_t own_w = w.own_w, mid_w = w.mid_w, last_w = w.last_w;
    if (prm.lambda1 != T(0)) {
      if (lane_ok) {
#pragma unroll
        for (int a = 0; a < P; ++a) {
          s0[own_w + a * L::A] = ua[a];
          s1[own_w + a * L::A] = ua[a];
        }
      }
      facet_sync<P>();
      if (lane_ok) {
        T x[P], y[P];
#pragma unroll
        for (int m = 0; m < P; ++m) x[m] = s1[last_w + m];
        facet_line<T, P, false, FacetParams<T>>(dm, x, y);
#pragma unroll
        for (int m = 0; m < P; ++m) s1[last_w + m] = y[m];
      }
      if (lane_ok) {
        T x[P], y[P];
#pragma unroll
        for (int m = 0; m < P; ++m) x[m] = s0[mid_w + m * L::B];
        facet_line<T, P, false, FacetParams<T>>(dm, x, y);
// ... 75 lines not shown
      }
      facet_sync<P>();
      if (lane_ok) {
#pragma unroll
        for (int a = 0; a < P; ++a) {
          const T v = s0[own_w + a * L::A] + s1[own_w + a * L::A];
          if (GM == GEO_AFFINE) acc[a] += v;
          else acc[a] += prm.lambda1 * v;
        }
      }
      if (GM == GEO_POINT && MASS && lane_ok) {
#pragma unroll
        for (int a = 0; a < P; ++a) {
          T G[6], Wm;
          geom.factors(dm, a, false, true, G, Wm);
          acc[a] += prm.lambda0 * Wm * ua[a];
        }
      }
      facet_sync<P>();
    } else {
#pragma unroll
      for (int a = 0; a < P; ++a) acc[a] = T(0);
      if (MASS && lane_ok) {
#pragma unroll
        for (int a = 0; a < P; ++a) {
          if constexpr (GM == GEO_AFFINE) {
            acc[a] = (Wm0 * sym_w<T, P>(dm, a)) * ua[a];
          } else {
            T G[6], Wm;
            geom.factors(dm, a, false, true, G, Wm);
            acc[a] = prm.lambda0 * Wm * ua[a];
          }
        }
      }
    }
  }
};

template <typename T, int P, bool MASS>
struct BoxElem {
  using L = FacetLayout<P>;
  using Mat = SMat<T, P>;
  static constexpr int CODE_WORDS =
      (L::COPY * 4 + (int)sizeof(T) - 1) / (int)sizeof(T);
  static constexpr int LDS_WORDS = L::COPY + CODE_WORDS;
  static constexpr int MINW = P >= 9 ? SFEM_FACET_BOX_MINW_HI : SFEM_FACET_BOX_MINW;
  static constexpr int CHAIN_MINW =
      P >= 9 ? SFEM_FACET_CHAIN_MINW_HI : SFEM_FACET_CHAIN_MINW_BOX;
  static constexpr bool CHAINS = true;
  static constexpr bool LAYERED_SLOTS = P <= 8;
  struct Raw { T c[4]; };
  T P0, P1, P2, Wm;

  static __device__ __forceinline__ void fetch(Raw& raw,
                                               const FacetParams<T>& prm,
                                               int64_t e) {
    const T* g = prm.geo_const + e * 8;
    raw.c[0] = g[0]; raw.c[1] = g[3]; raw.c[2] = g[5]; raw.c[3] = g[6];
  }
  __device__ __forceinline__ void finish(const Raw& raw,
                                         const FacetParams<T>& prm,
                                         const Mat& sm, const Mat* ksm,
                                         const FacetWave<P>& w, T wij) {
    const T wi = ksm->w[w.i], wj = ksm->w[w.j];
    P0 = prm.lambda1 * raw.c[0] * wij;
    P1 = prm.lambda1 * raw.c[1] * wj;
    P2 = prm.lambda1 * raw.c[2] * wi;
    Wm = MASS ? prm.lambda0 * raw.c[3] * wij : T(0);
  }

  __device__ __forceinline__ void apply(const FacetParams<T>& prm,
                                        const Mat& sm, const FacetWave<P>& w,
                                        T* lds, const T (&ua)[P],
                                        T (&acc)[P]) const {
    T* s0 = lds;
    const bool lane_ok = w.ok;
    const uint32_t own_w = w.own_w, mid_w = w.mid_w, last_w = w.last_w;
    if (prm.lambda1 != T(0)) {
      if (lane_ok) {
#pragma unroll
        for (int a = 0; a < P; ++a) s0[own_w + a * L::A] = ua[a];
      }
      {
        T r0[P];
        facet_sym_line<T, P, FacetParams<T>>(sm, ua, r0);
#pragma unroll
        for (int a = 0; a < P; ++a) {
          acc[a] = P0 * r0[a];
          if (MASS) acc[a] += (Wm * ua[a]) * sym_w<T, P>(sm, a);
        }
      }
      facet_sync<P>();
      T y1[P];
      {
        T x[P], y2[P];
#pragma unroll
        for (int m = 0; m < P; ++m) x[m] = lane_ok ? s0[last_w + m] : T(0);
        facet_sym_line<T, P, FacetParams<T>>(sm, x, y2);
#pragma unroll
        for (int m = 0; m < P; ++m)
          x[m] = lane_ok ? s0[mid_w + m * L::B] : T(0);
        facet_sync<P>();
        if (lane_ok) {
#pragma unroll
          for (int m = 0; m < P; ++m) s0[last_w + m] = y2[m];
        }
        facet_sym_line<T, P, FacetParams<T>>(sm, x, y1);
      }
      facet_sync<P>();
#pragma unroll
      for (int a = 0; a < P; ++a) {
// ... 45 lines not shown
  {
    typename ELEM::Raw raw;
    ELEM::fetch(raw, prm, e);
    el.finish(raw, prm, dm, kdm, w, w.template wij<T>(kdm));
  }

  const int nc = SCALAR ? 1 : prm.ncomp;
  double udot = 0.0;
  for (int k = 0; k < nc; ++k) {
    const T* ug = prm.u + (SCALAR ? 0 : k * prm.comp_stride);
    T* og = prm.out + (SCALAR ? 0 : k * prm.comp_stride);
    T ua[P], acc[P];
    if (w.ok) {
#pragma unroll
      for (int a = 0; a < P; ++a) {
        ua[a] = *facet_node<const T, OFF32>(ug, fl.code(a));
      }
    } else {
#pragma unroll
      for (int a = 0; a < P; ++a) ua[a] = T(0);
    }
    el.apply(prm, dm, w, lds, ua, acc);
    if (w.ok)
      facet_scatter_head<T, P, LAY>(fl, acc, ua, prm.dot_out != nullptr, udot);
    if constexpr (LAY && !ELEM::LAYERED_SLOTS) {
      facet_store_layered<T, P, OFF32>(fl, acc, og, w.ok);
    } else {
      uint16_t slots[6];
#pragma unroll
      for (int q = 0; q < 6; ++q) slots[q] = g_facet_slots<P>.s[w.lane][q];
      if constexpr (LAY)
        facet_store_layered_slots<T, P, OFF32>(
            fl, slots, acc, og, s0, codes, w.own_w, w.ok,
            FacetLane<P>::cls(w.i) == 1 && FacetLane<P>::cls(w.j) == 1);
      else
        facet_scatter_tail<T, P, OFF32>(fl, slots, acc, og, s0, codes, w.own_w,
                                        w.ok);
      facet_sync<P>();
    }
  }
  if (prm.dot_out) {
#pragma unroll
    for (int off = 32; off > 0; off >>= 1) udot += __shfl_down(udot, off, 64);
    if ((w.lane & 63) == 0) {
      const int64_t wave = (int64_t)blockIdx.x * L::WAVES + (w.lane >> 6);
      if (LAY && prm.dot_slots > 0)
        prm.dot_out[wave] = udot;
      else
        unsafeAtomicAdd(&prm.dot_out[wave & (SFEM_DOT_SLOTS - 1)], udot);
    }
  }
}

template <typename T, int P, typename ELEM, bool OFF32, bool LAY = false>
__global__ void __launch_bounds__(FacetLayout<P>::BLOCK, ELEM::CHAIN_MINW)
helmholtz_chain_kernel(FacetParams<T> prm, typename ELEM::Mat dm) {
  using L = FacetLayout<P>;
  using Mat = typename ELEM::Mat;
  using KA = FacetKernarg<FacetParams<T>, Mat>;
  using FL = FacetLane<P, LAY>;
  __shared__ T lds[ELEM::LDS_WORDS];
  T* s0 = lds;
  uint32_t* codes = reinterpret_cast<uint32_t*>(lds + L::COPY);

  FacetWave<P> w;
  w.init();
  const uint32_t seg = blockIdx.x;
  const int32_t k0 = prm.chain_off[seg];
  const int32_t k1 = prm.chain_off[seg + 1];
  const Mat* kdm = reinterpret_cast<const Mat*>(kernarg_bytes() + KA::MAT_OFF);
  constexpr bool OWN_ORDER = LAY && !ELEM::LAYERED_SLOTS;
  uint16_t slots[OWN_ORDER ? 1 : 6];
  if constexpr (!OWN_ORDER) {
#pragma unroll
    for (int q = 0; q < 6; ++q) slots[q] = g_facet_slots<P>.s[w.lane][q];
  }
  const bool face_inner = FL::cls(w.i) == 1 && FL::cls(w.j) == 1;
  const T* ug = prm.u;
  T* og = prm.out;

  const T wij = w.template wij<T>(kdm);
  double udot = 0.0;
  T carry = T(0);
  {
  FL fl, fn;
  typename FL::Raw traw;
  typename ELEM::Raw graw;
  fl.load(prm.tab, (int64_t)prm.chain_elems[k0], w.i, w.j);
  fn = fl;
  ELEM::fetch(graw, prm, (int64_t)prm.chain_elems[k0]);
  T ua[P];
#pragma unroll
  for (int a = 0; a < P; ++a)
    ua[a] = w.ok ? *facet_node<const T, OFF32>(ug, fl.code(a)) : T(0);
  if (k0 + 1 < k1)
    FL::issue(traw, prm.tab, (int64_t)prm.chain_elems[k0 + 1], w.i, w.j);
  for (int32_t k = k0; k < k1; ++k) {
    const bool has_pred = k > k0, has_succ = k + 1 < k1;
    ELEM el;
    el.finish(graw, prm, dm, kdm, w, wij);
    if (has_succ) {
      fn.finish(traw, w.i, w.j);
      ELEM::fetch(graw, prm, (int64_t)prm.chain_elems[k + 1]);
    }
    T acc[P];
    el.apply(prm, dm, w, lds, ua, acc);
    if (has_pred) acc[0] += carry;
    carry = acc[P - 1];
    FL fe = fl;
    if constexpr (LAY) {
      if (has_succ) fe.to[2] |= FACET_SKIP | SFEM_IDX_DIRICHLET;
    } else {
      if (has_pred && face_inner) fe.t[0] &= ~(uint32_t)SFEM_IDX_SHARED;
      if (has_succ) fe.t[2] |= SFEM_IDX_SHARED | SFEM_IDX_DIRICHLET;
    }
    const T u_last = ua[P - 1];
    if (w.ok)
      facet_scatter_head<T, P, LAY>(fe, acc, ua, prm.dot_out != nullptr, udot);
    fl = fn;
    if (has_succ) {
      ua[0] = u_last;
#pragma unroll
      for (int a = 1; a < P; ++a)
        ua[a] = w.ok ? *facet_node<const T, OFF32>(ug, fl.code(a)) : T(0);
      if (k + 2 < k1)
        FL::issue(traw, prm.tab, (int64_t)prm.chain_elems[k + 2], w.i, w.j);
    }
    if constexpr (OWN_ORDER) {
      facet_store_layered<T, P, OFF32>(fe, acc, og, w.ok);
    } else {
      if constexpr (LAY)
        facet_store_layered_slots<T, P, OFF32>(fe, slots, acc, og, s0, codes,
                                               w.own_w, w.ok, face_inner);
      else
        facet_scatter_tail<T, P, OFF32>(fe, slots, acc, og, s0, codes, w.own_w,
                                        w.ok);
      facet_sync<P>();
    }
  }
  }
  if (prm.dot_out) {
#pragma unroll
    for (int off = 32; off > 0; off >>= 1) udot += __shfl_down(udot, off, 64);
    if ((w.lane & 63) == 0) {
      const int64_t wave = (int64_t)blockIdx.x * L::WAVES + (w.lane >> 6);
      if (LAY && prm.dot_slots > 0)
        prm.dot_out[wave] = udot;
      else
        unsafeAtomicAdd(&prm.dot_out[wave & (SFEM_DOT_SLOTS - 1)], udot);
    }
  }
}

template <typename T>
inline bool facet_off32(int64_t field_reals) {
  const char* force64 = getenv("SFEM_FACET_OFF64");
  return (uint64_t)field_reals * sizeof(T) < ((uint64_t)1 << 32) &&
         !(force64 && force64[0] == '1');
}

template <typename T, int P, typename ELEM>
int launch_facet_elem(const FacetParams<T>& prm, const typename ELEM::Mat& mat,
                      unsigned groups, bool off32, hipStream_t stream) {
  const dim3 grid(groups), block(FacetLayout<P>::BLOCK);
  if (prm.layered && prm.ncomp != 1) {
    set_error("helmholtz (facet): layered assembly takes scalar fields");
    return SFEM_EINVAL;
  }
  if (prm.chain_off && !ELEM::CHAINS) {
    set_error("helmholtz (facet): no chain kernel for this geometry at P=%d",
              P);
    return SFEM_EUNSUPPORTED;
  }
  with_flag(off32, [&](auto o32) {
    constexpr bool O32 = decltype(o32)::value;
    if (prm.chain_off) {
      if constexpr (ELEM::CHAINS) {
        if (prm.layered)
          hipLaunchKernelGGL((helmholtz_chain_kernel<T, P, ELEM, O32, true>),
                             grid, block, 0, stream, prm, mat);
        else
          hipLaunchKernelGGL((helmholtz_chain_kernel<T, P, ELEM, O32>), grid,
                             block, 0, stream, prm, mat);
      }
    } else if (prm.layered) {
      hipLaunchKernelGGL((helmholtz_facet_kernel<T, P, ELEM, true, O32, true>),
                         grid, block, 0, stream, prm, mat);
    } else if (prm.ncomp == 1) {
      hipLaunchKernelGGL((helmholtz_facet_kernel<T, P, ELEM, true, O32>), grid,
                         block, 0, stream, prm, mat);
    } else {
      hipLaunchKernelGGL((helmholtz_facet_kernel<T, P, ELEM, false, O32>),
                         grid, block, 0, stream, prm, mat);
    }
  });
  return SFEM_OK;
}

template <typename T, int P>
int launch_helmholtz_facet(const FacetParams<T>& prm, int geo_mode,
                           int64_t groups, int64_t field_reals,
                           const T* dmat, const T* weights, const T* nodes,
                           hipStream_t stream) {
  if (int rc = check_groups("helmholtz (facet)", groups)) return rc;
  if (prm.chain_off && prm.ncomp != 1) {
    set_error("helmholtz (facet): chain launches take scalar fields");
    return SFEM_EINVAL;
  }
  const unsigned g = (unsigned)groups;
  if (prm.dot_out && prm.layered && prm.dot_slots > 0 &&
      groups * FacetLayout<P>::WAVES > prm.dot_slots) {
    set_error("helmholtz (facet): %lld waves but %lld dot slots",
              (long long)(groups * FacetLayout<P>::WAVES),
              (long long)prm.dot_slots);
    return SFEM_EINVAL;
  }
  const bool off32 = facet_off32<T>(field_reals);
  int rc = SFEM_OK;
  with_flag(prm.lambda0 != T(0), [&](auto mass) {
    constexpr bool MASS = decltype(mass)::value;
    if (geo_mode == GEO_BOX) {
      const SMat<T, P> sm = make_smat<T, P>(dmat, weights);
      rc = launch_facet_elem<T, P, BoxElem<T, P, MASS>>(prm, sm, g, off32,
                                                        stream);
// ... 61 lines not shown
```

swirl_fem_amd/linalg/cg.py:

```python

from __future__ import annotations

from typing import NamedTuple

import torch

from swirl_fem_amd import switches
from swirl_fem_amd import _lib
from swirl_fem_amd import _ops
from swirl_fem_amd.core import layout
from swirl_fem_amd.linalg import _driver


def _leaves(t):
  if isinstance(t, dict):
    return [l for k in sorted(t) for l in _leaves(t[k])]
  if isinstance(t, (list, tuple)):
    return [l for x in t for l in _leaves(x)]
  return [t]


def _map(f, *ts):
  t0 = ts[0]
  if isinstance(t0, dict):
    return {k: _map(f, *[t[k] for t in ts]) for k in t0}
  if isinstance(t0, (list, tuple)):
    return type(t0)(_map(f, *xs) for xs in zip(*ts))
  return f(*ts)


def _as_vec(t):
  if not isinstance(t, torch.Tensor):
    raise TypeError(f'cg operates on device tensors, got {type(t)}')
  return t


MAX_KEPT_RUNNERS = 6
LAZY_X_MIN_BYTES = 1 << 28
RR_PARTIALS = 1 << 16
RESIDUAL_STOP_GROUPS = 512
FUSE_RR_SPREAD = 2


def _lazy_min_bytes():
  mb = switches.get('SFEM_LAZY_X_MIN_MB')
  return LAZY_X_MIN_BYTES if mb is None else int(float(mb) * (1 << 20))


_ResidualStop = NamedTuple('_ResidualStop', [
    ('groups', int), ('layered', object), ('parts', torch.Tensor),
    ('waves', torch.Tensor), ('num_waves', int)])
_Mean = NamedTuple('_Mean', [('w', torch.Tensor), ('total', float),
                             ('sums', torch.Tensor)])
_Jacobi = NamedTuple('_Jacobi', [('dinv', torch.Tensor), ('ncomp', int)])
_Det = NamedTuple('_Det', [('wave_sums', torch.Tensor),
                           ('rr_sums', torch.Tensor)])
_Lazy = NamedTuple('_Lazy', [('ring', torch.Tensor), ('n', int),
                             ('state', torch.Tensor)])


class _Scalars:
  GAMMA, PAP, GAMMA_NEW, ALPHA, BETA, BB, ATOL2, DONE, ITERS = range(9)
  STATUS = 10

  def __init__(self, device):
    self.t = torch.zeros(_lib.SFEM_CG_NSCALARS, dtype=torch.float64,
                         device=device)
    self.partials = torch.zeros(_lib.SFEM_DOT_SLOTS, dtype=torch.float64,
                                device=device)

  def interface_correction(self, slot, a, b, interface):
    idx, w = interface
    if idx.numel() == 0:
      return
    for x, y in zip(_leaves(a), _leaves(b)):
      _ops.dot_indexed(x, layout.like(y, x), idx, w, self.t, slot, -1.0)

  def complete(self, slot, a, b, reduce_fn, interface):
    if interface is not None:
      self.interface_correction(slot, a, b, interface)
    if reduce_fn is not None:
      reduce_fn(self.t[slot:slot + 1])

  def dot_into(self, slot, a, b, dot_fn, reduce_fn, interface=None,
               cleared=False):
    la, lb = _leaves(a), _leaves(b)
    if dot_fn is None:
      first = not cleared
      for x, y in zip(la, lb):
        _ops.dot(layout.flat(x), layout.flat(layout.like(y, x)), self.t, slot,
                 accumulate=not first)
        first = False
    else:
      total = sum(dot_fn(x, y) for x, y in zip(la, lb))
      self.t[slot] = torch.as_tensor(total, dtype=torch.float64,
                                     device=self.t.device)
    self.complete(slot, a, b, reduce_fn, interface)


class CGRunner:

  def __init__(self, A, b, x0=None, *, tol=1e-5, atol=0.0, maxiter=None,
               M=None, dot_fn=None, reduce_fn=None, interface=None):
    if interface is not None and (
        dot_fn is not None or
        (M is not None and not getattr(M, 'consistent', False))):
      raise ValueError('interface weights apply to the plain dot of consistent '
                       'vectors (M = None or a preconditioner that maps '
                       'consistent vectors to consistent ones, dot_fn = None)')
    b_leaves = [_as_vec(l) for l in _leaves(b)]
    if not all(l.is_cuda for l in b_leaves):
      raise RuntimeError('swirl_fem_amd.linalg.cg runs on MI355X device '
                         'tensors (there is no CPU fallback)')
    self.A, self.M, self.dot_fn, self.reduce_fn = A, M, dot_fn, reduce_fn
    self.interface = interface
    self.tol, self.atol = tol, atol
    if maxiter is None:
      maxiter = 10 * sum(l.numel() for l in b_leaves)
    self.maxiter = maxiter
    dense = lambda t: t if (t.is_contiguous() or
                            layout.is_component_major(t)) else t.contiguous()
    b = _map(dense, b)
    self._x = (_map(torch.zeros_like, b) if x0 is None
               else _map(lambda t, bb: layout.like(t, bb).clone(), x0, b))
    self.s = _Scalars(b_leaves[0].device)
    self.identity_m = M is None
    self.issued = 0
    self._graph = None
    self._capture_failed = False
    z = self._start_vectors(b, allocate=True)
    self.fused_dot = (dot_fn is None and hasattr(A, 'apply_with_dot') and
                      isinstance(self._p, torch.Tensor))
    self.fuse_rr = FUSE_RR_SPREAD if self.identity_m and dot_fn is None else 0
    self.fold_rr = bool(self.fuse_rr) and (reduce_fn is not None or
                                           interface is not None)
    self.parts = self.s.partials if self.fused_dot else None
    self._start_scalars(z)
    self.rr_stop = self._select_residual_stop()
    if self.rr_stop is not None:
      self.fused_dot, self.parts = False, None
    self._args = (self.maxiter, self.tol, self.atol, self.parts)
    self.merged = self.fused_dot and reduce_fn is None
    self.mean = self._select_mean()
    self.jacobi = self._select_jacobi()
    self.jacobi_interface = None
    if self.jacobi is not None and interface is not None:
      idx, w = interface
      self.jacobi_interface = (
          idx, (w * self.jacobi.dinv[idx].double()).contiguous())
    self.layered = self._select_layered()
    self.det = self._select_det()
    self.lazy = self._select_lazy()
    self._start_fixed_order_sums(b, z)

  def _select_residual_stop(self):
    A = self.A
    if not (getattr(self.M, 'stops_on_residual', False) and
            self.dot_fn is None and isinstance(self.r, torch.Tensor) and
            self.r.dim() == 1):
      return None
    dev = self.r.device
    G = RESIDUAL_STOP_GROUPS
    layered = None
    if (hasattr(A, 'apply_layered_with_dot') and hasattr(A, 'layer_plan') and
        self.reduce_fn is None and self.interface is None):
      layered = A.layer_plan()
    waves = A.layered_dot_slots() if layered is not None else 0
    return _ResidualStop(
        groups=G, layered=layered,
        parts=torch.zeros(2 * G, dtype=torch.float64, device=dev),
        waves=torch.zeros(waves + _lib.SFEM_FOLD_GROUPS, dtype=torch.float64,
                          device=dev), num_waves=waves)

  def _select_mean(self):
    probe = getattr(self.M, 'mean_projection', None)
    if not (probe is not None and self.rr_stop is None and
            self.dot_fn is None and self.reduce_fn is None and
            self.interface is None and isinstance(self.r, torch.Tensor) and
            switches.get('SFEM_FUSED_MEAN') != '0'):
      return None
    found = probe()
    if found is None:
      return None
    w, total = found
    return _Mean(layout.flat(layout.like(w.to(self.r.dtype), self.r)),
                 float(total),
                 torch.zeros(_lib.SFEM_CG_MEAN_SUMS, dtype=torch.float64,
                             device=self.r.device))

  def _select_jacobi(self):
    probe = getattr(self.M, 'jacobi_diagonal', None)
    r = self.r
    if not (probe is not None and self.mean is None and
            self.rr_stop is None and self.dot_fn is None and
            (self.interface is not None or self.reduce_fn is None) and
            isinstance(r, torch.Tensor) and
            switches.get('SFEM_FUSED_JACOBI') != '0'):
      return None
    dinv = probe()
    dinv = None if dinv is None else dinv.to(r.dtype).contiguous()
    n = -1 if dinv is None else dinv.numel()
    vn = 16 // r.element_size()
    if r.dim() == 1 or (r.dim() == 2 and r.shape[1] == 1 and
                        r.is_contiguous()):
      ncomp = 1
    elif (r.dim() == 2 and layout.is_component_major(r) and
          self._p.stride() == r.stride() and n % vn == 0):
      ncomp = r.shape[1]
    else:
      return None
    return _Jacobi(dinv, ncomp) if r.shape[0] == n else None

  def _select_layered(self):
    if (self.fused_dot and self.mean is None and self.rr_stop is None and
        self._p.dim() == 1 and hasattr(self.A, 'apply_layered_with_dot')):
      return self.A.layer_plan()
    return None

  def _select_det(self):
    if not (self.layered is not None and self.reduce_fn is None and
            self.interface is None and
            switches.get('SFEM_DETERMINISTIC') != '0'):
      return None
    pad = _lib.SFEM_FOLD_GROUPS
    dev = self.r.device
    return _Det(torch.zeros(self.A.layered_dot_slots() + pad,
                            dtype=torch.float64, device=dev),
                torch.zeros(RR_PARTIALS + pad, dtype=torch.float64,
                            device=dev))

  def _select_lazy(self):
    m = int(switches.get('SFEM_LAZY_X'))
    p = self._p
    if not (m >= 2 and self.mean is None and self.jacobi is None and
            self.rr_stop is None and isinstance(p, torch.Tensor) and
            p.is_contiguous() and
            p.numel() * p.element_size() >= _lazy_min_bytes()):
      return None
    m = min(m, _lib.SFEM_CG_LAZY_MAX)
    n = p.numel()
    ring = torch.empty((m, (n + 3) // 4 * 4), dtype=p.dtype, device=p.device)
    ring[0, :n] = p.reshape(-1)
    self._p = None
    self._shape = tuple(self.r.shape)
    return _Lazy(ring, n, torch.zeros(1 + _lib.SFEM_CG_LAZY_MAX,
                                      dtype=torch.float64, device=p.device))

  def _start_vectors(self, b, allocate=False):
    s, S = self.s, _Scalars
    s.dot_into(S.BB, b, b, self.dot_fn, self.reduce_fn, self.interface)
    Ax = self.A(self._x)
    if allocate:
      self.r = _map(lambda bb, ax: bb - layout.like(ax, bb), b, Ax)
    else:
      _map(lambda rr, bb, ax: rr.copy_(layout.like(bb, rr) -
                                       layout.like(ax, rr)), self.r, b, Ax)
    z = self.r if self.identity_m else self.M(self.r)
    if allocate:
      self._p = _map(lambda t, rr: layout.like(t, rr).clone(), z, self.r)
    else:
      _map(lambda pp, zz: pp.copy_(layout.like(zz, pp)), self.p, z)
    return z

  def _start_scalars(self, z):
    s = self.s
    s.dot_into(_Scalars.GAMMA, self.r, z, self.dot_fn, self.reduce_fn,
               self.interface)
    _ops.cg_scalars(s.t, 2, self.maxiter, self.tol, self.atol, self.parts)

  def _start_fixed_order_sums(self, b, z):
    if self.det is not None:
      self._reproducible_start(b, z)
    if self.rr_stop is not None:
      self._residual_stop_start(b, z)

  def _residual_stop_start(self, b, z):
    st = self.rr_stop
    args = (self.maxiter, self.tol, self.atol)
    self._dot2(b, b, None)
    _ops.pmg_cg_scalars(self.s.t, 3, st.parts, st.groups, *args)
    self._dot2(self.r, self.r, layout.like(z, self.r).contiguous())
    _ops.pmg_cg_scalars(self.s.t, 2, st.parts, st.groups, *args)

  def _dot2(self, a, b, c):
    G, parts = self.rr_stop.groups, self.rr_stop.parts
    _ops.pmg_dot2(a, b, c, parts, G)
    if self.interface is not None:
      idx, w = self.interface
      if idx.numel():
        _ops.dot_indexed(a, b, idx, w, parts, 0, -1.0)
        if c is not None:
          _ops.dot_indexed(a, c, idx, w, parts, G, -1.0)
    if self.reduce_fn is not None:
      self.reduce_fn(parts[:G if c is None else 2 * G])

  def _reproducible_start(self, b, z):
    s, S = self.s, _Scalars
    tree = lambda u, v: (u.double() * v.double()).sum()
    s.t[S.BB] = tree(b, b)
    s.t[S.GAMMA] = tree(self.r, z)
    _ops.cg_scalars(s.t, 2, self.maxiter, self.tol, self.atol, self.parts)

  @property
  def vector_passes(self):
    if self.jacobi is not None:
      return 10
    if self.lazy is None:
      return 8
    m = self.lazy.ring.shape[0]
    return 3 + (4 * m + 1) / m

  @property
  def p(self):
    if self.lazy is None:
      return self._p
    ring, n, _ = self.lazy
    return ring[self.issued % ring.shape[0], :n].view(self._shape)

  @property
  def x(self):
    if self.lazy is not None:
      self._flush()
      _ops.cg_flush_x(layout.flat(self._x), self.lazy.ring, self.s.t,
                      self.lazy.state)
    return self._x

  def matches(self, b, tol, atol, maxiter) -> bool:
    mine, theirs = _leaves(self.r), _leaves(b)
    if len(mine) != len(theirs) or (tol, atol) != (self.tol, self.atol):
      return False
    if maxiter is None:
      maxiter = 10 * sum(l.numel() for l in theirs)
    if maxiter != self.maxiter:
      return False
    return all(isinstance(t, torch.Tensor) and t.shape == m.shape and
               t.dtype == m.dtype and t.device == m.device and
               (t.stride() == m.stride() or t.is_contiguous())
               for m, t in zip(mine, theirs))

  def restart(self, b, x0=None):
    if x0 is None:
      _map(lambda xx: xx.zero_(), self._x)
    else:
      _map(lambda xx, t: xx.copy_(layout.like(t, xx)), self._x, x0)
    self.issued = 0
    if self.lazy is not None:
      self.lazy.state.zero_()
    z = self._start_vectors(b)
    self._start_scalars(z)
    self._start_fixed_order_sums(b, z)
    if self.mean is not None:
      self.mean.sums.zero_()

  def step(self):
    if self._graph is not None:
      self._graph.replay()
      self.issued += 1
      return
    self._step_eager()

  def _step_eager(self):
    if self.rr_stop is not None:
      self._step_residual_stop()
      return
    Ap = self._apply_and_alpha()
    z = self._update_r(Ap)
    self._update_xp(z)
    self._close()

  def _apply_and_alpha(self):
    s, S, A = self.s, _Scalars, self.A
    if self.det is not None:
      sums = self.det.wave_sums
      Ap = A.apply_layered_with_dot(self.p, sums, per_wave=True)
      _ops.cg_scalars_n(s.t, 5, self.maxiter, self.tol, self.atol, sums,
                        sums.numel() - _lib.SFEM_FOLD_GROUPS)
      return Ap
    if self.fused_dot:
      Ap = (A.apply_layered_with_dot(self.p, s.partials)
            if self.layered is not None
            else A.apply_with_dot(self.p, s.partials))
      _ops.cg_scalars(s.t, 5 if self.merged else 3, *self._args)
      if self.reduce_fn is not None:
        self.reduce_fn(s.t[S.PAP:S.PAP + 1])
    else:
      Ap = A(self.p)
      s.dot_into(S.PAP, self.p, Ap, self.dot_fn, self.reduce_fn,
                 self.interface, cleared=True)
    if not self.merged:
      _ops.cg_scalars(s.t, 0, *self._args)
    return Ap

  def _update_r(self, Ap):
    s, S, M = self.s, _Scalars, self.M
    if self.mean is not None:
      _ops.cg_update_r_mean(layout.flat(self.r),
                            layout.flat(layout.like(Ap, self.r)), self.mean.w,
                            s.t, self.mean.sums)
      return None
    if self.jacobi is not None:
      self._update_r_jacobi(Ap)
      return None
    plan = self.layered
    if plan is not None and self.det is not None and self.fuse_rr:
      n = _ops.cg_update_r_layered_det(
          self.r, Ap, plan.layers, s.t, self.det.rr_sums[:RR_PARTIALS],
          masks=plan.masks)
      _ops.cg_scalars_n(s.t, 8, self.maxiter, self.tol, self.atol,
                        self.det.rr_sums, n)
    elif plan is not None:
      _ops.cg_update_r_layered(self.r, Ap, plan.layers, s.t, self.fuse_rr,
                               masks=plan.masks)
    else:
      for rr, aa in zip(_leaves(self.r), _leaves(Ap)):
        _ops.cg_update_r(layout.flat(rr), layout.flat(layout.like(aa, rr)),
                         s.t, self.fuse_rr)
    if self.fuse_rr:
      if self.fold_rr:
        _ops.cg_scalars(s.t, 7, *self._args)
        s.complete(S.GAMMA_NEW, self.r, self.r, self.reduce_fn,
                   self.interface)
      return self.r
    if (self.dot_fn is None and hasattr(M, 'apply_with_dot') and
        isinstance(self.r, torch.Tensor)):
      z = M.apply_with_dot(self.r, s.t, S.GAMMA_NEW)
      s.complete(S.GAMMA_NEW, self.r, z, self.reduce_fn, self.interface)
    else:
      z = self.r if self.identity_m else M(self.r)
      s.dot_into(S.GAMMA_NEW, self.r, z, self.dot_fn, self.reduce_fn,
                 self.interface, cleared=True)
    return z

  def _update_r_jacobi(self, Ap):
    s, plan = self.s, self.layered
    dinv, ncomp = self.jacobi
    if plan is None:
      r, Ap = layout.flat(self.r), layout.flat(layout.like(Ap, self.r))
      layers, masks = (), None
    else:
      r, layers, masks = self.r, plan.layers, plan.masks
    sums = (self.det.rr_sums[:RR_PARTIALS]
            if plan is not None and self.det is not None else None)
    n = _ops.cg_update_r_jacobi(r, Ap, dinv, s.t, ncomp, layers, masks, sums)
    if sums is not None:
      _ops.cg_scalars_n(s.t, 8, self.maxiter, self.tol, self.atol,
                        self.det.rr_sums, n)
    if self.reduce_fn is not None:
      _ops.cg_scalars(s.t, 7, *self._args)
      s.complete(_Scalars.GAMMA_NEW, self.r, self.r, self.reduce_fn,
                 self.jacobi_interface)

  def _update_xp(self, z):
    s = self.s
    if self.mean is not None:
      _ops.cg_update_xp_mean(layout.flat(self._x), layout.flat(self.p),
                             layout.flat(self.r), s.t, self.mean.sums,
                             self.mean.total)
    elif self.jacobi is not None:
      dinv, ncomp = self.jacobi
      _ops.cg_update_xp_jacobi(layout.flat(self._x), layout.flat(self.p),
                               layout.flat(self.r), dinv, s.t, ncomp)
    elif self.lazy is not None:
      _ops.cg_update_xp_lazy(layout.flat(self._x), self.lazy.ring,
                             layout.flat(layout.like(z, self.r)), s.t,
                             self.lazy.state)
    else:
      for xx, pp, zz in zip(_leaves(self._x), _leaves(self.p), _leaves(z)):
        _ops.cg_update_xp(layout.flat(xx), layout.flat(pp),
                          layout.flat(layout.like(zz, pp)), s.t)

  def _close(self):
    if not self.merged:
      _ops.cg_scalars(self.s.t, 1, *self._args)
    self.issued += 1

  def _step_residual_stop(self):
    s, st = self.s, self.rr_stop
    G, parts = st.groups, st.parts
    args = (self.maxiter, self.tol, self.atol)
    if st.layered is not None:
      Ap = self.A.apply_layered_with_dot(self.p, st.waves, per_wave=True)
      _ops.pmg_cg_scalars(s.t, 0, st.waves, st.num_waves, *args)
      _ops.cg_update_r_layered(self.r, Ap, st.layered.layers, s.t, 0,
                               masks=st.layered.masks)
    else:
      Ap = layout.like(self.A(self.p), self.r).contiguous()
      self._dot2(self.p, Ap, None)
      _ops.pmg_cg_scalars(s.t, 0, parts, G, *args)
      _ops.cg_update_r(self.r, Ap, s.t, 0)
    z = layout.like(self.M(self.r), self.r).contiguous()
    self._dot2(self.r, self.r, z)
    _ops.pmg_cg_scalars(s.t, 4, parts, G, *args)
    _ops.cg_update_xp(self._x, self.p, z, s.t)
    _ops.pmg_cg_scalars(s.t, 1, parts, G, *args)
    self.issued += 1

  def capture(self) -> bool:
    if self._graph is not None:
      return True
    if self.reduce_fn is not None:
      return False
    if self.lazy is not None:
      if self.issued:
        return False
      ring, n, _ = self.lazy
      self._p = ring[0, :n].view(self._shape).clone()
      self.lazy = None
    self.step()
    torch.cuda.synchronize()
    issued = self.issued
    self._graph = _driver.capture_graph(self._step_eager)
    self.issued = issued
    if self._graph is None:
      self._capture_failed = True
    return self._graph is not None

  def _flush(self):
    if self.merged:
      _ops.cg_scalars(self.s.t, 6, self.maxiter, self.tol, self.atol, None)

  def done(self) -> bool:
    self._flush()
    return bool(self.s.t[_Scalars.DONE].item() != 0.0)

  def info(self):
    self._flush()
    scal = self.s.t.cpu()
    status = _lib.CG_STATUS.get(int(scal[_Scalars.STATUS].item()), 'unknown')
    if status == 'running' and self.issued >= self.maxiter:
      status = 'maxiter'
    return {'residual': self.s.t[_Scalars.GAMMA].clone(),
            'num_iterations': int(scal[_Scalars.ITERS].item()),
            'status': status}


def cg(A, b, x0=None, *, tol=1e-5, atol=0.0, maxiter=None, M=None,
       dot_fn=None, reduce_fn=None, interface=None, check_every=16,
       graph=False, workspace=None, key=None):
  if not _leaves(b):
    return b, {'residual': 0.0, 'num_iterations': 0, 'status': 'converged'}
  reuse = (graph and workspace is not None and key is not None and
           dot_fn is None and reduce_fn is None and interface is None)
  run, kept = _driver.kept_runner(
      workspace if reuse else None, key, MAX_KEPT_RUNNERS,
      lambda run: run.matches(b, tol, atol, maxiter),
      lambda: CGRunner(A, b, x0, tol=tol, atol=atol, maxiter=maxiter, M=M,
                       dot_fn=dot_fn, reduce_fn=reduce_fn,
                       interface=interface))
  if kept:
    run.restart(b, x0)
  if (graph and dot_fn is None and run.maxiter > 2 and run._graph is None and
      not run._capture_failed and not run.done()):
    run.capture()
  _driver.drive(run, check_every)
  info = run.info()
  _driver.warn_on_breakdown('cg', info)
  return (_map(lambda t: t.clone(), run.x) if reuse else run.x), info


class _SymmetricSolve(torch.autograd.Function):

  @staticmethod
  def forward(ctx, b, A, kwargs, info_out):
    x, info = cg(A, b.detach(), **kwargs)
    if info_out is not None:
      info_out.update(info)
    ctx.A, ctx.kwargs = A, kwargs
    return x

  @staticmethod
# ... 8 lines not shown
```

swirl_fem_amd/switches.py:

```python

from __future__ import annotations

import os
import warnings

SWITCHES = {
    'SFEM_LIB': (None, '_lib.py',
                 'path of another build of libsfem_hip.so (kernel A/B runs, '
                 '`scripts/build_variant.sh`)'),
    'SFEM_HDF5_LIB': (None, 'niles/datagen/h5lite.py',
                      'path of the HDF5 C library for snapshot files when '
                      'h5py is not installed'),
    'SFEM_FACET': ('1', 'core/operators.py',
                   '0: 3D P = 6..12 operators keep their index rows instead '
                   'of the compact facet tables'),
    'SFEM_BOX': ('1', 'core/operators.py',
                 '0: Cartesian elements run the general affine kernels'),
    'SFEM_CHAIN': ('1', 'core/operators.py, _ops.py',
                   '0: one element per wave instead of chain segments'),
    'SFEM_CHAIN_LEN': (None, 'core/operators.py',
                       'elements per chain segment (default: 8 on large '
                       'meshes, shorter on small ones, '
                       '`operators.chain_segment_length`)'),
    'SFEM_CHAIN_HI': ('0', 'core/operators.py',
                      '1: chains also for P >= 9 box / affine elements '
                      '(slower: measured 1.73 vs 1.47 ms at p = 11)'),
    'SFEM_CHAIN_VECTOR': ('1', '_ops.py',
                          '0: component-major vector fields are not walked '
                          'as chains'),
    'SFEM_LAYERED': ('1', 'core/operators.py',
                     '0: CG keeps the atomic assembly; force: layered '
                     'assembly also for elements with stored factors'),
    'SFEM_DETERMINISTIC': ('1', 'linalg/cg.py',
                           '0: with layered assembly the two inner products '
                           'of a CG iteration still accumulate their partial '
                           'sums with atomics (not bitwise reproducible; one '
                           'scalar launch less per iteration)'),
    'SFEM_LAZY_X': ('4', 'linalg/cg.py',
                    'directions the CG keeps before it adds them to x '
                    '(vectors of 256 MB and more; 0 or 1: x += alpha p every '
                    'iteration)'),
    'SFEM_LAZY_X_MIN_MB': (None, 'linalg/cg.py',
                           'smallest vector (MiB) that gets the lazy x update '
                           '(default 256; the tests set 0)'),
    'SFEM_SORTED_SCATTER': ('1', 'core/operators.py',
                            '0: index-row kernels issue their atomics in slot '
                            'order instead of node order'),
    'SFEM_CLUSTER': ('0', 'core/operators.py',
                     "1: assembly='auto' means cluster assembly (slower)"),
    'SFEM_INTERP': ('1', 'the library (getenv per launch)',
                    '0: values-only sfem_basis_eval / sfem_basis_eval_t run '
                    'the generic kernels instead of the compile-time-sized '
                    'interpolation (csrc/sfem_interp.h)'),
    'SFEM_MFMA': ('0', '_ops.py and the library (getenv per launch)',
                  '1: p = 11 fp32 index-row elements run the matrix-core '
                  'kernel (slower: 1.25 vs 1.0 ms)'),
    'SFEM_FACET_OFF64': ('0', 'the library (getenv per launch)',
                         '1: facet kernels form 64-bit addresses even for '
                         'fields below 4 GiB (tests)'),
    'SFEM_STOKES_FACET': ('1', 'core/operators.py',
                          '0: Stokes div / grad_t keep their index rows'),
    'SFEM_STOKES_FACET_DIV': ('box', 'core/operators.py',
                              'all: the divergence walks chains on every '
                              'geometry, not only on box elements (tests)'),
    'SFEM_SPLIT_E': ('0', 'navier_stokes/navier_stokes.py',
                     '1: pressure operator E in two fused halves '
                     '(`sfem_stokes_e_first/second`)'),
    'SFEM_STOKES_LAYERED': ('auto', 'navier_stokes/navier_stokes.py',
                            'pressure operator E on index-row kernels: D^T '
                            'with one position per writer instead of atomics '
                            '(`StokesDivGrad.e_layered`); auto = 2D meshes, '
                            '1 = 3D index rows too, 0 = never'),
    'SFEM_FUSED_DOTS': ('1', 'navier_stokes/navier_stokes.py',
                        '0: the pressure CG computes p.Ep and r.Mr with '
                        'separate dot kernels'),
    'SFEM_FUSED_MEAN': ('1', 'linalg/cg.py',
                        '0: the mean projection of the pressure '
                        'preconditioner is applied as a separate kernel'),
    'SFEM_FUSED_JACOBI': ('1', 'linalg/cg.py',
                          '0: a Jacobi preconditioner (`linalg/jacobi.py`) is '
                          'called as a function and z = M r stored, instead '
                          'of being folded into the two CG vector updates'),
    'SFEM_GRAPHS': ('1', 'navier_stokes/navier_stokes.py',
                    '0: solver iterations are never replayed as HIP graphs'),
    'SFEM_GRAPH_REUSE': ('1', 'navier_stokes/navier_stokes.py',
                         '0: a recorded iteration is not kept across solves'),
    'SFEM_GRAPH_MAX_NUMEL': (str(1 << 25), 'navier_stokes/navier_stokes.py',
                             'largest vector (entries) whose solves are '
                             'replayed as graphs'),
    'SFEM_PRESSURE_PC': ('projection', 'examples/navier_stokes_driver.py',
                         "pressure preconditioner of the drivers: 'projection' "
                         "(the reference's nullspace projection) or 'schwarz' "
                         '(element-wise fast diagonalisation + piecewise-'
                         'constant coarse level, '
                         'navier_stokes/pressure_preconditioner.py)'),
    'SFEM_VELOCITY_PC': ('exchange', 'navier_stokes/navier_stokes.py',
                         "preconditioner of the stepper's Helmholtz solve: "
# ... 71 lines not shown
```

Measured before the change: 67.27.

## Form interior CG direction entries inside the layered chain operator apply

The lazy x/p update now writes the new direction only for surface (non-element-interior) nodes. The interior entries p = z + beta*p_old are computed on the fly inside the layered chain Helmholtz kernel as it gathers them, and a small finish kernel completes them only when p is needed elsewhere. The aim is to drop one full write and re-read of most of the direction vector per iteration at high order, where interior nodes dominate. In exchange the chain kernel gets a new direction-forming template variant with extra register pressure and a node-ordering requirement checked at plan build time.

Result: faster. 69.60, median of 4 (+3.5%).

```diff
diff --git a/include/sfem.h b/include/sfem.h
--- a/include/sfem.h
+++ b/include/sfem.h
@@ -376,6 +376,19 @@
 int sfem_cg_flush_x(void* x, const void* pring, int64_t ring_stride,
                     int64_t count, const double* scalars, double* lazy, int m,
                     int dtype, sfem_stream_t stream);
+int sfem_cg_update_xp_lazy_split(void* x, void* pring, int64_t ring_stride,
+                                 const void* z, int64_t count,
+                                 int64_t direction_count, double* scalars,
+                                 double* lazy, int m, int dtype,
+                                 sfem_stream_t stream);
+int sfem_cg_finish_direction(void* p_new, const void* p_old, const void* z,
+                             int64_t begin, int64_t count,
+                             const double* scalars, int dtype,
+                             sfem_stream_t stream);
+int sfem_helmholtz_apply_direction(const sfem_helmholtz_args* args,
+                                   const void* r, const void* p_old,
+                                   const double* scalars,
+                                   sfem_stream_t stream);
 #define SFEM_MAX_LAYERS 15
 #define SFEM_LAYER_CHUNK 512
 int sfem_cg_update_r_layered(void* r, const void* ap_ext, int64_t count,
diff --git a/swirl_fem_amd/_lib.py b/swirl_fem_amd/_lib.py
--- a/swirl_fem_amd/_lib.py
+++ b/swirl_fem_amd/_lib.py
@@ -252,6 +252,12 @@
                                c_i32, c_i32, c_ptr],
     'sfem_cg_flush_x': [c_ptr, c_ptr, c_i64, c_i64, c_ptr, c_ptr, c_i32, c_i32,
                         c_ptr],
+    'sfem_cg_update_xp_lazy_split': [c_ptr, c_ptr, c_i64, c_ptr, c_i64, c_i64,
+                                     c_ptr, c_ptr, c_i32, c_i32, c_ptr],
+    'sfem_cg_finish_direction': [c_ptr, c_ptr, c_ptr, c_i64, c_i64, c_ptr,
+                                 c_i32, c_ptr],
+    'sfem_helmholtz_apply_direction': [ctypes.POINTER(HelmholtzArgs), c_ptr,
+                                       c_ptr, c_ptr, c_ptr],
     'sfem_cg_update_r_mean': [c_ptr, c_ptr, c_ptr, c_i64, c_ptr, c_ptr, c_i32,
                               c_ptr],
     'sfem_cg_update_xp_mean': [c_ptr, c_ptr, c_ptr, c_i64, c_ptr, c_ptr, c_dbl,
diff --git a/swirl_fem_amd/_ops.py b/swirl_fem_amd/_ops.py
--- a/swirl_fem_amd/_ops.py
+++ b/swirl_fem_amd/_ops.py
@@ -575,12 +575,21 @@
 
 
 def helmholtz_apply_layered(u, ext, enc, parts, host, ndim, P, lambda0,
-                            lambda1, dot_out=None, per_wave=False):
+                            lambda1, dot_out=None, per_wave=False,
+                            direction=None):
   dev = _dev(enc)
   if u.dim() != 1 or not u.is_contiguous() or not ext.is_contiguous():
     raise ValueError('layered assembly takes contiguous scalar fields')
   if ext.dtype != u.dtype:
     raise ValueError('u and the extended output differ in dtype')
+  if direction is not None:
+    r, p_old, dir_scalars = direction
+    if len(parts) != 1 or not parts[0].get('layered_chains'):
+      raise ValueError('the direction is formed by ONE layered chain launch')
+    if not (r.is_contiguous() and p_old.is_contiguous() and
+            r.dtype == p_old.dtype == u.dtype and
+            r.numel() == p_old.numel() == u.numel()):
+      raise ValueError('r and p_old must be contiguous vectors like u')
   host = {k: _host(v, u.dtype) for k, v in host.items()}
   waves = (layered_dot_waves(parts, P, enc.shape[0])
            if per_wave and dot_out is not None else None)
@@ -596,6 +605,11 @@
                              dot_slots=0 if waves is None else waves[n])
       if waves is not None:
         at += waves[n]
+      if direction is not None:
+        _lib.check(_lib.load().sfem_helmholtz_apply_direction(
+            ctypes.byref(args), _ptr(r), _ptr(p_old), _ptr(dir_scalars),
+            _stream(dev)), 'sfem_helmholtz_apply_direction')
+        continue
       _lib.check(_lib.load().sfem_helmholtz_apply(ctypes.byref(args),
                                                   _stream(dev)),
                  'sfem_helmholtz_apply')
@@ -1390,13 +1404,28 @@
         _dtype_code(r), _stream(dev)), 'sfem_cg_update_r')
 
 
-def cg_update_xp_lazy(x, pring, z, scalars, lazy):
+def cg_update_xp_lazy(x, pring, z, scalars, lazy, direction_count=None):
   dev = _dev(x, pring, z, scalars, lazy)
   with torch.cuda.device(dev):
-    _lib.check(_lib.load().sfem_cg_update_xp_lazy(
-        _ptr(x), _ptr(pring), pring.stride(0), _ptr(z), x.numel(),
-        _ptr(scalars), _ptr(lazy), pring.shape[0], _dtype_code(x),
-        _stream(dev)), 'sfem_cg_update_xp_lazy')
+    if direction_count is None:
+      _lib.check(_lib.load().sfem_cg_update_xp_lazy(
+          _ptr(x), _ptr(pring), pring.stride(0), _ptr(z), x.numel(),
+          _ptr(scalars), _ptr(lazy), pring.shape[0], _dtype_code(x),
+          _stream(dev)), 'sfem_cg_update_xp_lazy')
+    else:
+      _lib.check(_lib.load().sfem_cg_update_xp_lazy_split(
+          _ptr(x), _ptr(pring), pring.stride(0), _ptr(z), x.numel(),
+          int(direction_count), _ptr(scalars), _ptr(lazy), pring.shape[0],
+          _dtype_code(x), _stream(dev)), 'sfem_cg_update_xp_lazy_split')
+
+
+def cg_finish_direction(p_new, p_old, z, begin, scalars):
+  dev = _dev(p_new, p_old, z, scalars)
+  with torch.cuda.device(dev):
+    _lib.check(_lib.load().sfem_cg_finish_direction(
+        _ptr(p_new), _ptr(p_old), _ptr(z), int(begin), p_new.numel(),
+        _ptr(scalars), _dtype_code(p_new), _stream(dev)),
+        'sfem_cg_finish_direction')
 
 
 def cg_flush_x(x, pring, scalars, lazy):
diff --git a/swirl_fem_amd/core/operators.py b/swirl_fem_amd/core/operators.py
--- a/swirl_fem_amd/core/operators.py
+++ b/swirl_fem_amd/core/operators.py
@@ -237,6 +237,38 @@
   num_nodes: int
   masks: tuple | None = None
   read: int = 0
+  interior_begin: int | None = None
+
+
+def interior_split(table, num_nodes, P):
+  M = P - 2
+  if M < 1 or table.numel() == 0:
+    return None
+  t = table.to(torch.int64)
+  E = t.shape[0]
+  id0 = (t[..., 0] & 0xFFFFFFFF) & 0x3FFFFFFF
+  strides = t[..., 1:]
+  f = torch.arange(27, device=t.device)
+  inner = torch.stack([f // 9 == 1, (f // 3) % 3 == 1, f % 3 == 1], dim=1)
+  span = strides * (M - 1) * inner[None].to(torch.int64)
+  lo = id0 + span.clamp(max=0).sum(-1)
+  hi = id0 + span.clamp(min=0).sum(-1) + 1
+  INTERIOR = 13
+  mags = torch.sort(strides[:, INTERIOR].abs(), dim=1).values
+  want = torch.tensor([1, M, M * M], device=t.device)
+  if M > 1 and not bool((mags == want[None]).all()):
+    return None
+  ilo, order = torch.sort(lo[:, INTERIOR])
+  ihi = hi[:, INTERIOR][order]
+  n_s = int(ilo[0])
+  if (not bool((ihi - ilo == M ** 3).all()) or int(ihi[-1]) != num_nodes or
+      not bool((ilo[1:] == ihi[:-1]).all())):
+    return None
+  other = torch.ones(27, dtype=torch.bool, device=t.device)
+  other[INTERIOR] = False
+  if int(hi[:, other].max()) > n_s:
+    return None
+  return n_s
 
 
 def build_layer_plan(facet_parts, num_elements, num_nodes, P):
@@ -327,8 +359,13 @@
     bytes_.append(m)
     read += min(int(m.sum()) * chunk, ln)
   masks = (torch.cat(bytes_), moffs) if bytes_ else None
+  n_s = None
+  if (len(parts) == 1 and parts[0]['layered_chains'] and P <= 8 and
+      'elem_list' not in parts[0]):
+    n_s = interior_split(tab, N, P)
   return LayerPlan(layers=list(zip(lens, offs)), extent=extent, parts=parts,
-                   written=written, num_nodes=N, masks=masks, read=read)
+                   written=written, num_nodes=N, masks=masks, read=read,
+                   interior_begin=n_s)
 
 
 def _cluster_limits(fespace):
@@ -924,20 +961,26 @@
                        device=self.enc.device)
 
   def apply_layered(self, u, ext, lambda0=0.0, lambda1=1.0, *, dot_out=None,
-                    per_wave=False):
+                    per_wave=False, direction=None):
     plan = self.layer_plan()
     if plan is None:
       raise NotImplementedError('this operator has no layer plan')
+    if direction is not None and plan.interior_begin is None:
+      raise NotImplementedError('this layer plan cannot form the direction')
     mesh = self.fespace.mesh
     if tuple(u.shape) != (mesh.num_nodes,):
       raise ValueError(f'expected ({mesh.num_nodes},) nodal values, got '
                        f'{tuple(u.shape)}')
     if tuple(ext.shape) != (plan.extent,):
       raise ValueError(f'expected an extended output of {plan.extent} values')
+    if direction is not None and not (u.dtype == self.fespace.dtype and
+                                      u.is_contiguous()):
+      raise ValueError('the direction is formed in place: u must be a '
+                       'contiguous vector of the operator\'s dtype')
     return _ops.helmholtz_apply_layered(
         u.to(self.fespace.dtype).contiguous(), ext, self.enc, plan.parts,
         self.host, mesh.ndim, mesh.gridpoints_1d.num_points, lambda0, lambda1,
-        dot_out, per_wave)
+        dot_out, per_wave, direction)
 
   def layered_dot_slots(self):
     mesh = self.fespace.mesh
@@ -1038,6 +1081,8 @@
 
 class FusedLinearOperator:
 
+  forms_direction = True
+
   def __init__(self, op, lambda0, lambda1):
     self.op, self.lambda0, self.lambda1 = op, lambda0, lambda1
     self._ext = None
@@ -1055,11 +1100,13 @@
       return None
     return plan
 
-  def apply_layered_with_dot(self, u, partials, per_wave=False):
+  def apply_layered_with_dot(self, u, partials, per_wave=False,
+                             direction=None):
     if self._ext is None:
       self._ext = self.op.new_extended()
     return self.op.apply_layered(u, self._ext, self.lambda0, self.lambda1,
-                                 dot_out=partials, per_wave=per_wave)
+                                 dot_out=partials, per_wave=per_wave,
+                                 direction=direction)
 
   def layered_dot_slots(self):
     return self.op.layered_dot_slots()
diff --git a/swirl_fem_amd/csrc/sfem_common.h b/swirl_fem_amd/csrc/sfem_common.h
--- a/swirl_fem_amd/csrc/sfem_common.h
+++ b/swirl_fem_amd/csrc/sfem_common.h
@@ -60,4 +60,18 @@
   return static_cast<unsigned>(blocks);
 }
 
+__device__ __forceinline__ double fma_real(double a, double b, double c) {
+  return __builtin_fma(a, b, c);
 }
+__device__ __forceinline__ float fma_real(float a, float b, float c) {
+  return __builtin_fmaf(a, b, c);
+}
+
+__device__ __forceinline__ double cg_gamma_new(const double* scalars) {
+  double v = scalars[SFEM_CG_NSCALARS_NAMED + (threadIdx.x & 63)];
+#pragma unroll
+  for (int off = 32; off > 0; off >>= 1) v += __shfl_xor(v, off, 64);
+  return scalars[2] + v;
+}
+
+}
diff --git a/swirl_fem_amd/csrc/sfem_core.hip b/swirl_fem_amd/csrc/sfem_core.hip
--- a/swirl_fem_amd/csrc/sfem_core.hip
+++ b/swirl_fem_amd/csrc/sfem_core.hip
@@ -388,12 +388,6 @@
   if (threadIdx.x == 0 && total != 0.0) unsafeAtomicAdd(result, scale * total);
 }
 
-__device__ __forceinline__ double cg_gamma_new(const double* scalars) {
-  double v = scalars[SFEM_CG_NSCALARS_NAMED + (threadIdx.x & 63)];
-#pragma unroll
-  for (int off = 32; off > 0; off >>= 1) v += __shfl_xor(v, off, 64);
-  return scalars[2] + v;
-}
 
 template <typename T, bool FUSE_RR>
 __global__ void __launch_bounds__(512)
@@ -550,7 +544,8 @@
 __global__ void __launch_bounds__(512)
 cg_update_xp_lazy_kernel(T* __restrict__ x, T* __restrict__ pring,
                          int64_t ring_stride, const T* __restrict__ z,
-                         int64_t count, const double* __restrict__ scalars,
+                         int64_t count, int64_t pcount,
+                         const double* __restrict__ scalars,
                          double* __restrict__ lazy, int m) {
   if (scalars[7] != 0.0) return;
   using V = typename Vec16<T>::type;
@@ -578,10 +573,15 @@
   V* pn = reinterpret_cast<V*>(pring + next * ring_stride);
   const V* zv = reinterpret_cast<const V*>(z);
   const int64_t stride = (int64_t)gridDim.x * blockDim.x;
-  for (int64_t i = (int64_t)blockIdx.x * blockDim.x + threadIdx.x; i < nvec;
+  const int64_t pfull = pcount / VN;
+  int64_t pvec = (pcount + VN - 1) / VN;
+  if (pvec > nvec) pvec = nvec;
+  const int64_t end = flush ? nvec : pvec;
+  for (int64_t i = (int64_t)blockIdx.x * blockDim.x + threadIdx.x; i < end;
        i += stride) {
     const V pp = ld16<T, NT>(&pk[i]);
-    const V zz = ld16<T, NT>(&zv[i]);
+    V zz{};
+    if (i < pfull) zz = ld16<T, NT>(&zv[i]);
     if (flush) {
       V xx = ld16<T, NT>(&xv[i]);
       for (int q = 0; q < n_old; ++q) {
@@ -596,11 +596,20 @@
         reinterpret_cast<T*>(&xx)[c] += alpha * vget<T>(pp, c);
       st16<T, NT>(xx, &xv[i]);
     }
-    V np;
-#pragma unroll
-    for (int c = 0; c < VN; ++c)
-      reinterpret_cast<T*>(&np)[c] = vget<T>(zz, c) + beta * vget<T>(pp, c);
-    st16<T, NT>(np, &pn[i]);
+    if (i < pfull) {
+      V np;
+#pragma unroll
+      for (int c = 0; c < VN; ++c)
+        reinterpret_cast<T*>(&np)[c] =
+            fma_real(beta, vget<T>(pp, c), vget<T>(zz, c));
+      st16<T, NT>(np, &pn[i]);
+    } else if (i * VN < pcount) {
+#pragma unroll
+      for (int c = 0; c < VN; ++c)
+        if (i * VN + c < pcount)
+          pring[next * ring_stride + i * VN + c] =
+              fma_real(beta, vget<T>(pp, c), z[i * VN + c]);
+    }
   }
   if (blockIdx.x == 0 && threadIdx.x < count - nvec * VN) {
     const int64_t i = nvec * VN + threadIdx.x;
@@ -612,8 +621,22 @@
       xx += alpha * pi;
       x[i] = xx;
     }
-    pring[next * ring_stride + i] = z[i] + beta * pi;
-  }
+    if (i < pcount) pring[next * ring_stride + i] = fma_real(beta, pi, z[i]);
+  }
+}
+
+template <typename T>
+__global__ void __launch_bounds__(512)
+cg_finish_direction_kernel(T* __restrict__ pnew, const T* __restrict__ pold,
+                           const T* __restrict__ z, int64_t begin,
+                           int64_t count,
+                           const double* __restrict__ scalars) {
+  if (scalars[7] != 0.0) return;
+  const T beta = (T)(cg_gamma_new(scalars) / scalars[0]);
+  const int64_t stride = (int64_t)gridDim.x * blockDim.x;
+  for (int64_t i = begin + (int64_t)blockIdx.x * blockDim.x + threadIdx.x;
+       i < count; i += stride)
+    pnew[i] = fma_real(beta, pold[i], z[i]);
 }
 
 template <typename T>
@@ -1769,7 +1792,17 @@
                            const void* z, int64_t count, double* scalars,
                            double* lazy, int m, int dtype,
                            sfem_stream_t stream) {
-  SFEM_REQUIRE(count >= 0 && scalars && lazy,
+  return sfem_cg_update_xp_lazy_split(x, pring, ring_stride, z, count, count,
+                                      scalars, lazy, m, dtype, stream);
+}
+
+int sfem_cg_update_xp_lazy_split(void* x, void* pring, int64_t ring_stride,
+                                 const void* z, int64_t count,
+                                 int64_t direction_count, double* scalars,
+                                 double* lazy, int m, int dtype,
+                                 sfem_stream_t stream) {
+  SFEM_REQUIRE(count >= 0 && scalars && lazy && direction_count >= 0 &&
+                   direction_count <= count,
                "sfem_cg_update_xp_lazy: bad arguments");
   SFEM_REQUIRE(m >= 2 && m <= SFEM_CG_LAZY_MAX,
                "sfem_cg_update_xp_lazy: ring of %d directions (2..%d)", m,
@@ -1787,11 +1820,34 @@
     if (streams_past_caches(count, sizeof(T)))
       hipLaunchKernelGGL((cg_update_xp_lazy_kernel<T, true>), dim3(grid),
                          dim3(512), 0, as_stream(stream), (T*)x, (T*)pring,
-                         ring_stride, (const T*)z, count, scalars, lazy, m);
+                         ring_stride, (const T*)z, count, direction_count,
+                         scalars, lazy, m);
     else
       hipLaunchKernelGGL((cg_update_xp_lazy_kernel<T, false>), dim3(grid),
                          dim3(512), 0, as_stream(stream), (T*)x, (T*)pring,
-                         ring_stride, (const T*)z, count, scalars, lazy, m);
+                         ring_stride, (const T*)z, count, direction_count,
+                         scalars, lazy, m);
+  });
+  SFEM_LAUNCH_CHECK();
+  return SFEM_OK;
+}
+
+int sfem_cg_finish_direction(void* p_new, const void* p_old, const void* z,
+                             int64_t begin, int64_t count,
+                             const double* scalars, int dtype,
+                             sfem_stream_t stream) {
+  SFEM_REQUIRE(begin >= 0 && begin <= count && scalars,
+               "sfem_cg_finish_direction: bad arguments");
+  SFEM_REQUIRE(dtype == SFEM_F32 || dtype == SFEM_F64,
+               "sfem_cg_finish_direction: unknown dtype %d", dtype);
+  if (begin == count) return SFEM_OK;
+  SFEM_REQUIRE(p_new && p_old && z && p_new != p_old,
+               "sfem_cg_finish_direction: null pointer or p_new = p_old");
+  DISPATCH_DTYPE(dtype, {
+    hipLaunchKernelGGL((cg_finish_direction_kernel<T>),
+                       dim3(stream_grid(count - begin, 512)), dim3(512), 0,
+                       as_stream(stream), (T*)p_new, (const T*)p_old,
+                       (const T*)z, begin, count, scalars);
   });
   SFEM_LAUNCH_CHECK();
   return SFEM_OK;
diff --git a/swirl_fem_amd/csrc/sfem_helmholtz.hip b/swirl_fem_amd/csrc/sfem_helmholtz.hip
--- a/swirl_fem_amd/csrc/sfem_helmholtz.hip
+++ b/swirl_fem_amd/csrc/sfem_helmholtz.hip
@@ -235,6 +235,9 @@
   int coef_mode = 0;
   const void* beta = nullptr;
   int adv_transpose = 0;
+  const void* dir_r = nullptr;
+  const void* dir_p = nullptr;
+  const double* dir_scalars = nullptr;
 };
 
 template <typename T>
@@ -295,6 +298,9 @@
     fp.chain_elems = c.chain_elems;
     fp.layered = c.layered_extent > 0;
     fp.dot_slots = c.dot_slots;
+    fp.dir_r = (const T*)c.dir_r;
+    fp.dir_p = (const T*)c.dir_p;
+    fp.dir_scalars = c.dir_scalars;
     if (fp.layered)
       return dispatch_helmholtz_facet<T>(
           fp, c.P, c.geo_mode,
@@ -444,7 +450,9 @@
   return SFEM_OK;
 }
 
-int sfem_helmholtz_apply(const sfem_helmholtz_args* a, sfem_stream_t stream) {
+static int helmholtz_apply(const sfem_helmholtz_args* a, const void* dir_r,
+                           const void* dir_p, const double* dir_scalars,
+                           sfem_stream_t stream) {
   SFEM_REQUIRE(a, "sfem_helmholtz_apply: null args");
   SFEM_REQUIRE(a->num_elements >= 0 && a->num_nodes >= 0 && a->ncomp >= 1 &&
                    a->ncomp <= 8,
@@ -560,9 +568,33 @@
   }
   SFEM_REQUIRE(!a->layered_extent || a->facet_table,
                "sfem_helmholtz_apply: layered assembly needs a facet table");
+  if (dir_scalars) {
+    SFEM_REQUIRE(c.layered_extent && c.chain_offsets && a->P <= 8 &&
+                     !a->beta && a->coef_mode == SFEM_COEF_NONE &&
+                     !a->elem_list,
+                 "sfem_helmholtz_apply_direction: needs ONE layered chain "
+                 "launch over every element, P <= 8");
+    SFEM_REQUIRE(dir_r && dir_p && dir_p != a->u && dir_r != a->u,
+                 "sfem_helmholtz_apply_direction: r, p_old and u must be "
+                 "three vectors");
+    c.dir_r = dir_r;
+    c.dir_p = dir_p;
+    c.dir_scalars = dir_scalars;
+  }
   return with_real(a->dtype, [&](auto zero) {
     return run_helmholtz<decltype(zero)>(c, as_stream(stream));
   });
+}
+
+int sfem_helmholtz_apply(const sfem_helmholtz_args* a, sfem_stream_t stream) {
+  return helmholtz_apply(a, nullptr, nullptr, nullptr, stream);
+}
+
+int sfem_helmholtz_apply_direction(const sfem_helmholtz_args* a, const void* r,
+                                   const void* p_old, const double* scalars,
+                                   sfem_stream_t stream) {
+  SFEM_REQUIRE(scalars, "sfem_helmholtz_apply_direction: null scalars");
+  return helmholtz_apply(a, r, p_old, scalars, stream);
 }
 
 int sfem_kernarg_selftest(int32_t* bad, sfem_stream_t stream) {
diff --git a/swirl_fem_amd/csrc/sfem_helmholtz_facet.h b/swirl_fem_amd/csrc/sfem_helmholtz_facet.h
--- a/swirl_fem_amd/csrc/sfem_helmholtz_facet.h
+++ b/swirl_fem_amd/csrc/sfem_helmholtz_facet.h
@@ -25,6 +25,9 @@
   double* dot_out;
   int layered;
   int64_t dot_slots;
+  const T* dir_r;
+  const T* dir_p;
+  const double* dir_scalars;
 };
 
 constexpr uint32_t FACET_SKIP = 0x40000000u;
@@ -43,6 +46,12 @@
     return A * x + B * y + z;
   }
 };
+
+template <bool KONST, typename V>
+__device__ __forceinline__ V facet_constant(const V* p, int64_t i) {
+  if constexpr (KONST) return ((const SFEM_CONSTANT_AS V*)p)[i];
+  else return p[i];
+}
 
 template <int P>
 __device__ __forceinline__ void facet_sync() {
@@ -318,32 +327,52 @@
 }
 
 template <typename T, int P, bool OFF32>
+__device__ __forceinline__ void facet_store_layered_slots_own(
+    const FacetLane<P, true>& fl, const T (&acc)[P], T* og, T* vals,
+    uint32_t* codes, uint32_t own_w, bool lane_ok, bool inner_lane) {
+  using L = FacetLayout<P>;
+  if (lane_ok && inner_lane) {
+#pragma unroll
+    for (int a = 1; a < P - 1; ++a)
+      *facet_node<T, OFF32>(og, fl.ocode(a)) = acc[a];
+  }
+  if (lane_ok) {
+#pragma unroll
+    for (int a = 0; a < P; ++a) {
+      vals[own_w + a * L::A] = acc[a];
+      codes[own_w + a * L::A] = fl.ocode(a);
+    }
+  }
+}
+
+template <typename T, int P, bool OFF32, bool PIN = false>
+__device__ __forceinline__ void facet_store_layered_slots_surface(
+    const uint16_t (&slots)[6], T* og, const T* vals, const uint32_t* codes,
+    int32_t tick = 0) {
+  facet_sync<P>();
+#pragma unroll
+  for (int q = 0; q < 6; ++q) {
+    uint32_t w = slots[q];
+    if (PIN) {
+      uint32_t pair = (uint32_t)slots[q & ~1] | ((uint32_t)slots[q | 1] << 16);
+      asm("" : "+v"(pair) : "s"(tick));
+      w = (q & 1) ? pair >> 16 : pair & 0xFFFFu;
+    }
+    if (w != 0xFFFFu) {
+      const uint32_t code = codes[w];
+      if (!(code & FACET_SKIP)) *facet_node<T, OFF32>(og, code) = vals[w];
+    }
+  }
+}
+
+template <typename T, int P, bool OFF32>
 __device__ __forceinline__ void facet_store_layered_slots(
     const FacetLane<P, true>& fl, const uint16_t (&slots)[6], const T (&acc)[P],
     T* og, T* vals, uint32_t* codes, uint32_t own_w, bool lane_ok,
     bool inner_lane) {
-  using L = FacetLayout<P>;
-  if (lane_ok && inner_lane) {
-#pragma unroll
-    for (int a = 1; a < P - 1; ++a)
-      *facet_node<T, OFF32>(og, fl.ocode(a)) = acc[a];
-  }
-  if (lane_ok) {
-#pragma unroll
-    for (int a = 0; a < P; ++a) {
-      vals[own_w + a * L::A] = acc[a];
-      codes[own_w + a * L::A] = fl.ocode(a);
-    }
-  }
-  facet_sync<P>();
-#pragma unroll
-  for (int q = 0; q < 6; ++q) {
-    const uint32_t w = slots[q];
-    if (w != 0xFFFFu) {
-      const uint32_t code = codes[w];
-      if (!(code & FACET_SKIP)) *facet_node<T, OFF32>(og, code) = vals[w];
-    }
-  }
+  facet_store_layered_slots_own<T, P, OFF32>(fl, acc, og, vals, codes, own_w,
+                                             lane_ok, inner_lane);
+  facet_store_layered_slots_surface<T, P, OFF32>(slots, og, vals, codes);
 }
 
 template <typename PRM, typename MAT>
@@ -458,14 +487,15 @@
   T lw, Wm0;
   ElemGeom<T, P, 3, (GM == GEO_AFFINE ? GEO_POINT : GM)> geom;
 
+  template <bool KONST = false>
   static __device__ __forceinline__ void fetch(Raw& raw,
                                                const FacetParams<T>& prm,
                                                int64_t e) {
     raw.e = e;
     if constexpr (GM == GEO_AFFINE) {
-      const T* g = prm.geo_const + e * 8;
-#pragma unroll
-      for (int q = 0; q < 7; ++q) raw.c[q] = g[q];
+#pragma unroll
+      for (int q = 0; q < 7; ++q)
+        raw.c[q] = facet_constant<KONST>(prm.geo_const, e * 8 + q);
     }
   }
   __device__ __forceinline__ void finish(const Raw& raw,
@@ -647,11 +677,15 @@
   struct Raw { T c[4]; };
   T P0, P1, P2, Wm;
 
+  template <bool KONST = false>
   static __device__ __forceinline__ void fetch(Raw& raw,
                                                const FacetParams<T>& prm,
                                                int64_t e) {
-    const T* g = prm.geo_const + e * 8;
-    raw.c[0] = g[0]; raw.c[1] = g[3]; raw.c[2] = g[5]; raw.c[3] = g[6];
+    const int64_t g = e * 8;
+    raw.c[0] = facet_constant<KONST>(prm.geo_const, g);
+    raw.c[1] = facet_constant<KONST>(prm.geo_const, g + 3);
+    raw.c[2] = facet_constant<KONST>(prm.geo_const, g + 5);
+    raw.c[3] = facet_constant<KONST>(prm.geo_const, g + 6);
   }
   __device__ __forceinline__ void finish(const Raw& raw,
                                          const FacetParams<T>& prm,
@@ -803,6 +837,65 @@
   }
 }
 
+
+__device__ __forceinline__ double wave_uniform(double v) {
+  return __hiloint2double(
+      __builtin_amdgcn_readfirstlane(__double2hiint(v)),
+      __builtin_amdgcn_readfirstlane(__double2loint(v)));
+}
+__device__ __forceinline__ float wave_uniform(float v) {
+  return __int_as_float(__builtin_amdgcn_readfirstlane(__float_as_int(v)));
+}
+
+template <typename T, int P, bool OFF32, bool DIR, int A0, typename FL>
+__device__ __forceinline__ void chain_gather(const FacetParams<T>& prm,
+                                             const FL& fl, bool ok,
+                                             bool dir_lane, T (&ua)[P],
+                                             T (&po)[DIR ? P : 1],
+                                             double& tie) {
+#pragma unroll
+  for (int a = A0; a < P; ++a) {
+    if (DIR && FL::cls(a) == 1) continue;
+    ua[a] = ok ? *facet_node<const T, OFF32>(prm.u, fl.code(a)) : T(0);
+  }
+  if constexpr (DIR) {
+    if (dir_lane) {
+#pragma unroll
+      for (int a = 1; a < P - 1; ++a) {
+        ua[a] = *facet_node<const T, OFF32>(prm.dir_r, fl.code(a));
+        po[a] = *facet_node<const T, OFF32>(prm.dir_p, fl.code(a));
+      }
+      asm("" : "+v"(tie));
+    } else {
+#pragma unroll
+      for (int a = 1; a < P - 1; ++a) {
+        ua[a] = ok ? *facet_node<const T, OFF32>(prm.u, fl.code(a)) : T(0);
+        po[a] = T(0);
+      }
+    }
+  }
+}
+
+template <typename T, int P, bool OFF32, typename FL>
+__device__ __forceinline__ void chain_form_direction(const FacetParams<T>& prm,
+                                                     const FL& fl,
+                                                     bool dir_lane, T beta,
+                                                     T (&ua)[P],
+                                                     const T (&po)[P]) {
+#pragma unroll
+  for (int a = 1; a < P - 1; ++a) {
+    const T v = fma_real(beta, po[a], ua[a]);
+    ua[a] = dir_lane ? v : ua[a];
+    asm("" : "+v"(ua[a]));
+  }
+  if (dir_lane) {
+    T* pn = const_cast<T*>(prm.u);
+#pragma unroll
+    for (int a = 1; a < P - 1; ++a)
+      *facet_node<T, OFF32>(pn, fl.code(a)) = ua[a];
+  }
+}
+
 template <typename T, int P, typename ELEM, bool OFF32, bool LAY = false>
 __global__ void __launch_bounds__(FacetLayout<P>::BLOCK, ELEM::CHAIN_MINW)
 helmholtz_chain_kernel(FacetParams<T> prm, typename ELEM::Mat dm) {
@@ -810,6 +903,7 @@
   using Mat = typename ELEM::Mat;
   using KA = FacetKernarg<FacetParams<T>, Mat>;
   using FL = FacetLane<P, LAY>;
+  constexpr bool DIR = LAY && L::WAVES == 1;
   __shared__ T lds[ELEM::LDS_WORDS];
   T* s0 = lds;
   uint32_t* codes = reinterpret_cast<uint32_t*>(lds + L::COPY);
@@ -827,32 +921,50 @@
     for (int q = 0; q < 6; ++q) slots[q] = g_facet_slots<P>.s[w.lane][q];
   }
   const bool face_inner = FL::cls(w.i) == 1 && FL::cls(w.j) == 1;
-  const T* ug = prm.u;
   T* og = prm.out;
 
   const T wij = w.template wij<T>(kdm);
+  T beta = T(0);
+  bool dir_lane = false;
+  if constexpr (DIR) {
+    if (prm.dir_scalars) {
+      beta = wave_uniform(
+          (T)(cg_gamma_new(prm.dir_scalars) / prm.dir_scalars[0]));
+      dir_lane = face_inner && prm.dir_scalars[7] == 0.0;
+    }
+  }
   double udot = 0.0;
   T carry = T(0);
   {
   FL fl, fn;
   typename FL::Raw traw;
   typename ELEM::Raw graw;
-  fl.load(prm.tab, (int64_t)prm.chain_elems[k0], w.i, w.j);
+  fl.load(prm.tab, (int64_t)facet_constant<DIR>(prm.chain_elems, k0), w.i,
+          w.j);
   fn = fl;
-  ELEM::fetch(graw, prm, (int64_t)prm.chain_elems[k0]);
-  T ua[P];
-#pragma unroll
-  for (int a = 0; a < P; ++a)
-    ua[a] = w.ok ? *facet_node<const T, OFF32>(ug, fl.code(a)) : T(0);
+  ELEM::template fetch<DIR>(
+      graw, prm, (int64_t)facet_constant<DIR>(prm.chain_elems, k0));
+  T ua[P], po[DIR ? P : 1];
+  chain_gather<T, P, OFF32, DIR, 0>(prm, fl, w.ok, dir_lane, ua, po, udot);
   if (k0 + 1 < k1)
-    FL::issue(traw, prm.tab, (int64_t)prm.chain_elems[k0 + 1], w.i, w.j);
+    FL::issue(traw, prm.tab,
+              (int64_t)facet_constant<DIR>(prm.chain_elems, k0 + 1), w.i, w.j);
   for (int32_t k = k0; k < k1; ++k) {
     const bool has_pred = k > k0, has_succ = k + 1 < k1;
+    if constexpr (DIR)
+      chain_form_direction<T, P, OFF32>(prm, fl, dir_lane, beta, ua, po);
     ELEM el;
-    el.finish(graw, prm, dm, kdm, w, wij);
+    if constexpr (DIR) {
+      const Mat* kd = kdm;
+      asm("" : "+s"(kd) : "s"(k));
+      el.finish(graw, prm, dm, kd, w, w.template wij<T>(kd));
+    } else {
+      el.finish(graw, prm, dm, kdm, w, wij);
+    }
     if (has_succ) {
       fn.finish(traw, w.i, w.j);
-      ELEM::fetch(graw, prm, (int64_t)prm.chain_elems[k + 1]);
+      ELEM::template fetch<DIR>(
+          graw, prm, (int64_t)facet_constant<DIR>(prm.chain_elems, k + 1));
     }
     T acc[P];
     el.apply(prm, dm, w, lds, ua, acc);
@@ -868,19 +980,29 @@
     const T u_last = ua[P - 1];
     if (w.ok)
       facet_scatter_head<T, P, LAY>(fe, acc, ua, prm.dot_out != nullptr, udot);
+    constexpr bool OWN_FIRST = DIR && !OWN_ORDER;
+    if constexpr (OWN_FIRST)
+      facet_store_layered_slots_own<T, P, OFF32>(fe, acc, og, s0, codes,
+                                                 w.own_w, w.ok, face_inner);
     fl = fn;
     if (has_succ) {
       ua[0] = u_last;
-#pragma unroll
-      for (int a = 1; a < P; ++a)
-        ua[a] = w.ok ? *facet_node<const T, OFF32>(ug, fl.code(a)) : T(0);
-      if (k + 2 < k1)
-        FL::issue(traw, prm.tab, (int64_t)prm.chain_elems[k + 2], w.i, w.j);
+      chain_gather<T, P, OFF32, DIR, 1>(prm, fl, w.ok, dir_lane, ua, po, udot);
+      if (k + 2 < k1) {
+        int ti = w.i, tj = w.j;
+        if constexpr (DIR) asm("" : "+v"(ti), "+v"(tj) : "s"(k));
+        FL::issue(traw, prm.tab,
+                  (int64_t)facet_constant<DIR>(prm.chain_elems, k + 2), ti,
+                  tj);
+      }
     }
     if constexpr (OWN_ORDER) {
       facet_store_layered<T, P, OFF32>(fe, acc, og, w.ok);
     } else {
-      if constexpr (LAY)
+      if constexpr (OWN_FIRST)
+        facet_store_layered_slots_surface<T, P, OFF32, true>(slots, og, s0,
+                                                             codes, k);
+      else if constexpr (LAY)
         facet_store_layered_slots<T, P, OFF32>(fe, slots, acc, og, s0, codes,
                                                w.own_w, w.ok, face_inner);
       else
@@ -921,6 +1043,11 @@
   if (prm.chain_off && !ELEM::CHAINS) {
     set_error("helmholtz (facet): no chain kernel for this geometry at P=%d",
               P);
+    return SFEM_EUNSUPPORTED;
+  }
+  if (prm.dir_scalars && !(prm.chain_off && prm.layered && P <= 8)) {
+    set_error("helmholtz (facet): the direction is formed by layered chain "
+              "launches at P <= 8 only");
     return SFEM_EUNSUPPORTED;
   }
   with_flag(off32, [&](auto o32) {
diff --git a/swirl_fem_amd/linalg/cg.py b/swirl_fem_amd/linalg/cg.py
--- a/swirl_fem_amd/linalg/cg.py
+++ b/swirl_fem_amd/linalg/cg.py
@@ -45,6 +45,13 @@
 def _lazy_min_bytes():
   mb = switches.get('SFEM_LAZY_X_MIN_MB')
   return LAZY_X_MIN_BYTES if mb is None else int(float(mb) * (1 << 20))
+
+
+def _fused_direction_min_bytes():
+  mb = switches.get('SFEM_FUSED_DIRECTION_MIN_MB')
+  if mb is None:
+    return LAZY_X_MIN_BYTES
+  return None if mb == 'off' else int(float(mb) * (1 << 20))
 
 
 _ResidualStop = NamedTuple('_ResidualStop', [
@@ -151,6 +158,8 @@
     self.layered = self._select_layered()
     self.det = self._select_det()
     self.lazy = self._select_lazy()
+    self.fused_dir = self._select_fused_direction()
+    self._dir_pending = False
     self._start_fixed_order_sums(b, z)
 
   def _select_residual_stop(self):
@@ -246,6 +255,26 @@
     return _Lazy(ring, n, torch.zeros(1 + _lib.SFEM_CG_LAZY_MAX,
                                       dtype=torch.float64, device=p.device))
 
+  def _select_fused_direction(self):
+    n_s = getattr(self.layered, 'interior_begin', None)
+    least = _fused_direction_min_bytes()
+    if not (n_s is not None and self.lazy is not None and least is not None and
+            self.merged and self.identity_m and self.reduce_fn is None and
+            self.interface is None and self.jacobi is None and
+            getattr(self.A, 'forms_direction', False) and
+            self.lazy.ring.shape[1] * self.lazy.ring.element_size() >= least):
+      return None
+    return int(n_s)
+
+  def _finish_direction(self):
+    if self._dir_pending:
+      ring, n, _ = self.lazy
+      m = ring.shape[0]
+      _ops.cg_finish_direction(ring[self.issued % m, :n],
+                               ring[(self.issued - 1) % m, :n],
+                               layout.flat(self.r), self.fused_dir, self.s.t)
+      self._dir_pending = False
+
   def _start_vectors(self, b, allocate=False):
     s, S = self.s, _Scalars
     s.dot_into(S.BB, b, b, self.dot_fn, self.reduce_fn, self.interface)
@@ -308,12 +337,19 @@
     if self.lazy is None:
       return 8
     m = self.lazy.ring.shape[0]
+    if self.fused_dir is not None:
+      s = self.fused_dir / self.lazy.n
+      return 3 + 3 * s + 2 * (1 - s) + (m + 1) / m
     return 3 + (4 * m + 1) / m
 
   @property
   def p(self):
     if self.lazy is None:
       return self._p
+    self._finish_direction()
+    return self._ring_p()
+
+  def _ring_p(self):
     ring, n, _ = self.lazy
     return ring[self.issued % ring.shape[0], :n].view(self._shape)
 
@@ -339,6 +375,7 @@
                for m, t in zip(mine, theirs))
 
   def restart(self, b, x0=None):
+    self._finish_direction()
     if x0 is None:
       _map(lambda xx: xx.zero_(), self._x)
     else:
@@ -370,14 +407,22 @@
 
   def _apply_and_alpha(self):
     s, S, A = self.s, _Scalars, self.A
+    kw = {}
+    if self._dir_pending:
+      ring, n, _ = self.lazy
+      kw['direction'] = (layout.flat(self.r),
+                         ring[(self.issued - 1) % ring.shape[0], :n], s.t)
+      self._dir_pending = False
     if self.det is not None:
       sums = self.det.wave_sums
-      Ap = A.apply_layered_with_dot(self.p, sums, per_wave=True)
+      Ap = A.apply_layered_with_dot(self._ring_p() if kw else self.p, sums,
+                                    per_wave=True, **kw)
       _ops.cg_scalars_n(s.t, 5, self.maxiter, self.tol, self.atol, sums,
                         sums.numel() - _lib.SFEM_FOLD_GROUPS)
       return Ap
     if self.fused_dot:
-      Ap = (A.apply_layered_with_dot(self.p, s.partials)
+      Ap = (A.apply_layered_with_dot(self._ring_p() if kw else self.p,
+                                     s.partials, **kw)
             if self.layered is not None
             else A.apply_with_dot(self.p, s.partials))
       _ops.cg_scalars(s.t, 5 if self.merged else 3, *self._args)
@@ -463,7 +508,8 @@
     elif self.lazy is not None:
       _ops.cg_update_xp_lazy(layout.flat(self._x), self.lazy.ring,
                              layout.flat(layout.like(z, self.r)), s.t,
-                             self.lazy.state)
+                             self.lazy.state, direction_count=self.fused_dir)
+      self._dir_pending = self.fused_dir is not None
     else:
       for xx, pp, zz in zip(_leaves(self._x), _leaves(self.p), _leaves(z)):
         _ops.cg_update_xp(layout.flat(xx), layout.flat(pp),
@@ -505,7 +551,7 @@
         return False
       ring, n, _ = self.lazy
       self._p = ring[0, :n].view(self._shape).clone()
-      self.lazy = None
+      self.lazy = self.fused_dir = None
     self.step()
     torch.cuda.synchronize()
     issued = self.issued
@@ -516,6 +562,7 @@
     return self._graph is not None
 
   def _flush(self):
+    self._finish_direction()
     if self.merged:
       _ops.cg_scalars(self.s.t, 6, self.maxiter, self.tol, self.atol, None)
 
diff --git a/swirl_fem_amd/switches.py b/swirl_fem_amd/switches.py
--- a/swirl_fem_amd/switches.py
+++ b/swirl_fem_amd/switches.py
@@ -43,6 +43,12 @@
     'SFEM_LAZY_X_MIN_MB': (None, 'linalg/cg.py',
                            'smallest vector (MiB) that gets the lazy x update '
                            '(default 256; the tests set 0)'),
+    'SFEM_FUSED_DIRECTION_MIN_MB': (None, 'linalg/cg.py',
+                                    'smallest vector (MiB) for which the '
+                                    'layered chain apply forms the element-'
+                                    'interior entries of the CG direction '
+                                    '(default 256, as the lazy x update; the '
+                                    'tests set 0; off: never)'),
     'SFEM_SORTED_SCATTER': ('1', 'core/operators.py',
                             '0: index-row kernels issue their atomics in slot '
                             'order instead of node order'),
```
